# TJUMMG/OCPG

Hardware: AMD Instinct MI355X
Metric: clips/sec fwd+bwd (5x384x640, R101) (higher is better)
Workload: dtype bf16

## Files before the change

include/ocpg_hip.h:

```cpp
#ifndef OCPG_HIP_H
#define OCPG_HIP_H
#include <stdint.h>

#ifdef __cplusplus
extern "C" {
#endif

int ocpg_msda_fwd_f32(const float* value, const int64_t* shapes, const int64_t* level_start,
                      const float* loc, const float* attn,
                      int N, int S, int M, int D, int L, int Lq, int P,
                      float* out, const int64_t* shapes_host, void* stream);
int ocpg_msda_fwd_f64(const double* value, const int64_t* shapes, const int64_t* level_start,
                      const double* loc, const double* attn,
                      int N, int S, int M, int D, int L, int Lq, int P,
                      double* out, void* stream);

int ocpg_msda_bwd_f32(const float* value, const int64_t* shapes, const int64_t* level_start,
                      const float* loc, const float* attn, const float* grad_out,
                      int N, int S, int M, int D, int L, int Lq, int P,
                      float* grad_value, float* grad_loc, float* grad_attn,
                      const int64_t* shapes_host, void* stream);
int ocpg_msda_bwd_value_f32(const float* loc, const float* attn, const float* grad_out,
                            int N, int S, int M, int D, int L, int Lq, int P,
                            float* grad_value, const int64_t* shapes_host, void* stream);
int ocpg_msda_bwd_locattn_f32(const float* value, const int64_t* shapes, const int64_t* level_start,
                              const float* loc, const float* attn, const float* grad_out,
                              int N, int S, int M, int D, int L, int Lq, int P,
                              float* grad_loc, float* grad_attn, void* stream);
int ocpg_msda_fused_fwd_f32(const float* value, const int64_t* shapes, const int64_t* level_start,
                            const float* qproj, const float* ref,
                            int N, int S, int M, int D, int L, int Lq, int P,
                            float* out, float* loc_out, float* attn_out, void* stream);
int ocpg_msda_fused_bwd_qproj_f32(const float* value, const int64_t* shapes, const int64_t* level_start,
                                  const float* loc, const float* attn, const float* grad_out,
                                  int N, int S, int M, int D, int L, int Lq, int P,
                                  float* grad_qproj, void* stream);
int ocpg_msda_bwd_value_sel_f32(const float* loc, const float* attn, const float* grad_out,
                                int N, int S, int M, int D, int L, int Lq, int P,
                                float* grad_value, const int64_t* shapes_host, int* sel_state, void* stream);
int ocpg_msda_bwd_f64(const double* value, const int64_t* shapes, const int64_t* level_start,
                      const double* loc, const double* attn, const double* grad_out,
                      int N, int S, int M, int D, int L, int Lq, int P,
                      double* grad_value, double* grad_loc, double* grad_attn, void* stream);

int ocpg_msda_fwd_h16(const void* value, const int64_t* shapes, const int64_t* level_start,
                      const float* loc, const float* attn,
                      int N, int S, int M, int D, int L, int Lq, int P,
                      void* out, const int64_t* shapes_host, int dtype, void* stream);
int ocpg_msda_bwd_h16(const void* value, const int64_t* shapes, const int64_t* level_start,
                      const float* loc, const float* attn, const void* grad_out,
                      int N, int S, int M, int D, int L, int Lq, int P,
                      float* grad_value, float* grad_loc, float* grad_attn,
                      const int64_t* shapes_host, int* sel_state, int dtype, void* stream);
int ocpg_msda_bwd_value_h16(const float* loc, const float* attn, const void* grad_out,
                            int N, int S, int M, int D, int L, int Lq, int P,
                            float* grad_value, const int64_t* shapes_host, int* sel_state, int dtype, void* stream);
int ocpg_msda_bwd_locattn_h16(const void* value, const int64_t* shapes, const int64_t* level_start,
                              const float* loc, const float* attn, const void* grad_out,
                              int N, int S, int M, int D, int L, int Lq, int P,
                              float* grad_loc, float* grad_attn, int dtype, void* stream);
int ocpg_msda_fused_fwd_h16(const void* value, const int64_t* shapes, const int64_t* level_start,
                            const float* qproj, const float* ref,
                            int N, int S, int M, int D, int L, int Lq, int P,
                            void* out, float* loc_out, float* attn_out, int dtype, void* stream);
int ocpg_msda_fused_bwd_qproj_h16(const void* value, const int64_t* shapes, const int64_t* level_start,
                                  const float* loc, const float* attn, const void* grad_out,
                                  int N, int S, int M, int D, int L, int Lq, int P,
                                  float* grad_qproj, int dtype, void* stream);

int ocpg_bn_act_fwd(const void* x, const float* scale, const float* shift, const void* skip, void* y,
                    long long n_outer, int C, long long inner, int relu, int dtype, void* stream);
int ocpg_bn_act_bwd(const void* gy, const void* y, const float* scale, void* gx, void* gskip,
                    long long n_outer, int C, long long inner, int relu, int dtype, void* stream);

int ocpg_gemm_dgrad_bn_tile(long long M, int N, int K);
int ocpg_gemm_dgrad_bn(const void* a, const void* w, const void* c, const void* mask, const float* scale, void* out, void* out_skip,
                       long long M, int N, int K, int dtype, int tile, void* stream);

int ocpg_win_attn_fwd(const void* qkv, const float* biasT, const int* region, float scale, int BW, int NW, int N, int H,
                      int head_dim, void* out, float* lse, int dtype, void* stream);
int ocpg_win_attn_bwd(const void* qkv, const float* bias, const float* biasT, const int* region, float scale, int BW, int NW,
                      int N, int H, int head_dim, const void* out, const void* dout, const float* lse, void* dqkv, float* Dbuf,
                      float* dbiasT, int dtype, void* stream);

int ocpg_win_attn_bwd_mfma(const void* qkv, const float* bias, const float* biasT, const int* region, float scale, int BW, int NW, int N,
                           int H, int head_dim, const void* out, const void* dout, const float* lse, void* dqkv, float* Dbuf, void* dS,
                           int dtype, void* stream);

int ocpg_win_attn_dtable_supported(int N, int head_dim, int dtype, int T);
int ocpg_win_attn_bwd_mfma_dtable(const void* qkv, const float* bias, const float* biasT, const int* region, float scale, int BW, int NW,
                                  int N, int H, int head_dim, const void* out, const void* dout, const float* lse, void* dqkv, float* Dbuf,
                                  const int* tok_code, int code_off, int T, float* partials, float* dtable, int dtype, void* stream);

int ocpg_dynmask_fwd_f32(const float* feats, const float* params, const float* refpix, int BT, int Q, int C, int H, int W,
                         int stride, float* out, float* pre1, void* stream);

int ocpg_dynmask_bwd_pre_f32(const float* dout, const float* pre1, const float* params, int BT, int Q, int C, int H, int W,
                             int stride, float* dpre, float* part, float* w0d, void* stream);
int ocpg_dynmask_bwd_fin_f32(const float* part, const float* params, const float* refpix, const float* dw0, int BT, int Q, int C,
                             int H, int W, float* dparams, float* dref, void* stream);

int ocpg_im2col3x3_nhwc(const void* x, int N, int H, int W, int C, int stride, int dil, void* cols, int dtype, void* stream);
int ocpg_col2im3x3_nhwc(const void* dcols, int N, int H, int W, int C, int stride, int dil, void* dx, int dtype, void* stream);

int ocpg_conv3x3_mfma_fwd(const void* x, const void* w, const float* scale, const float* bias, int relu, int N, int H, int W,
                          int Cin, int Cout, int stride, void* y, void* stream);
int ocpg_conv3x3_mfma_fwd_cols(const void* x, const void* w, const float* scale, const float* bias, int relu, int N, int H, int W, int Cin,
                               int Cout, int stride, void* y, void* cols, void* stream);
int ocpg_conv3x3_mfma_dgrad(const void* dy, const void* wT, int N, int H, int W, int Cin, int Cout, int stride, void* dx,
                            void* stream);
int ocpg_conv3x3_mfma_dgrad_masked(const void* dy, const void* wT, const void* mask_y, const float* scale, int N, int H, int W, int Cin,
                                   int Cout, int stride, void* dx, void* stream);
int ocpg_conv3x3_mfma_dgrad_w(const void* dy, const void* w, const void* mask_y, const float* scale, int N, int H, int W, int Cin, int Cout,
                              int stride, void* dx, void* stream);
int ocpg_conv3x3_mfma_body_splits(long long M, int ncols, int kchannels);
int ocpg_conv3x3_mfma_fwd_bn_splitk(const void* x, const void* w, const float* scale, const float* shift, int relu, int N, int H, int W, int Cin,
                                    int Cout, int stride, int splits, float* part, void* y, void* stream);
int ocpg_conv3x3_mfma_dgrad_w_splitk(const void* dy, const void* w, const void* mask_y, const float* scale, int N, int H, int W, int Cin,
                                     int Cout, int stride, int splits, float* part, void* dx, void* stream);
int ocpg_conv3x3_mfma_wgrad_splits(int N, int H, int W, int Cin, int Cout, int stride);
int ocpg_conv3x3_mfma_wgrad(const void* gz, const void* x, int N, int H, int W, int Cin, int Cout, int stride, void* part, void* stream);
int ocpg_conv3x3_mfma_fwd_cols_h16(const void* x, const void* w, const float* scale, const float* bias, int relu, int N, int H, int W, int Cin,
                                   int Cout, int stride, void* y, void* cols, int dtype, void* stream);
int ocpg_conv3x3_mfma_dgrad_w_h16(const void* dy, const void* w, const void* mask_y, const float* scale, int N, int H, int W, int Cin, int Cout,
                                  int stride, void* dx, int dtype, void* stream);
int ocpg_conv3x3_mfma_wgrad_h16(const void* gz, const void* x, int N, int H, int W, int Cin, int Cout, int stride, void* part, int dtype,
                                void* stream);

int ocpg_conv3x3_mfma_splits(int N, int H, int W, int Cin, int Cout, int stride);
int ocpg_conv3x3_mfma_fwd_splitk(const void* x, const void* w, const float* bias, int N, int H, int W, int Cin, int Cout, int stride,
                                 int splits, float* part, void* y, int out_dt, void* cols, void* stream);
int ocpg_conv3x3_mfma_fwd_splitk_h16(const void* x, const void* w, const float* bias, int N, int H, int W, int Cin, int Cout, int stride,
                                     int splits, float* part, void* y, int out_dt, void* cols, int dtype, void* stream);

int ocpg_gemm(const void* A, const void* B, void* C, const void* bias, int dtype, int out_dtype, int transA, int transB,
              long long M, long long N, long long K, long long lda, long long ldb, long long ldc, long long batch,
              long long strideA, long long strideB, long long strideC, float alpha, float beta, void* stream);
long long ocpg_gemm_plans(void);
long long ocpg_gemm_tuned(long long* changed);
long long ocpg_gemm_tune_rejected(void);
void ocpg_gemm_set_tuning(int on);
long long ocpg_gemm_export_picks(long long* buf, long long cap_pairs);
int ocpg_gemm_import_picks(const long long* buf, long long n_pairs);
int ocpg_gemm_bn_act(const void* A, const void* W, void* D, const float* scale, const float* shift, const void* skip, int relu, int dtype,
                     long long M, long long N, long long K, void* stream);

int ocpg_levelset_fwd_f32(const float* x, const float* feats, const float* box, int Lr, int N, int C, int CF, int h, int w, float* sums,
                          float* coef, float* loss, void* stream);
int ocpg_levelset_bwd_f32(const float* x, const float* feats, const float* box, const float* coef, const float* gloss, int Lr, int N,
                          int C, int CF, int h, int w, float* gx, float* gfeat, void* stream);
int ocpg_proj_fwd_f32(const float* x, const float* tcmax, const float* trmax, const float* tcmean, const float* trmean, int Lr, int B,
                      int T, int H, int W, float* colstat, float* rowstat, float* IU, float* loss, void* stream);
int ocpg_proj_bwd_f32(const float* x, const float* tcmax, const float* trmax, const float* tcmean, const float* trmean,
                      const float* colstat, const float* rowstat, const float* IU, const float* gloss, int Lr, int B, int T, int H, int W,
                      float* Gc, float* Gr, float* gx, void* stream);

int ocpg_matcher_cost_f32(const float* logits, const float* boxes, const float* masks, long long sl, long long sb, long long st,
                          long long sq, const float* gt, const float* tboxes, const float* valid, const long long* labels, int Lr,
                          int B, int T, int Q, int K, int h, int w, float wc, float wb, float wg, float wm, float wd, float* sums,
                          float* cost, int* bad, void* stream);

int ocpg_dropout_add_ln_fwd(const void* x, const float* res, const float* gamma, const float* beta, long long R, int C, float eps, float p,
                            unsigned long long seed, unsigned long long offset, const unsigned long long* rng_base, int x_dtype, float* y,
                            float* mean, float* rstd, void* stream);
int ocpg_dropout_add_ln_bwd(const float* gy, const void* x, const float* res, const float* gamma, const float* mean, const float* rstd,
                            long long R, int C, float p, unsigned long long seed, unsigned long long offset, const unsigned long long* rng_base,
                            int x_dtype, void* gx, float* gres, float* dgb_part, void* stream);
long long ocpg_dropout_add_ln_bwd_slots(long long R);
int ocpg_bias_relu_dropout_fwd(const void* a, const void* bias, long long R, int C, float p, unsigned long long seed,
                               unsigned long long offset, const unsigned long long* rng_base, int dtype, void* h, void* stream);
int ocpg_bias_relu_dropout_bwd(const void* gh, const void* h, long long R, int C, float p, int dtype, void* ga, float* dbias_part,
                               void* stream);
long long ocpg_bias_relu_dropout_bwd_slots(long long R, int C, int dtype);

int ocpg_multi_cast(const long long* srcs, const long long* dsts, const long long* numels, const long long* chunk_prefix, int n,
                    long long total_chunks, int src_dtype, int dst_dtype, void* stream);
int ocpg_multi_cast_sum(const long long* srcs, const long long* dsts, const long long* numels, const long long* chunk_prefix,
                        const long long* splits, const long long* strides, int n, long long total_chunks, int src_dtype, int dst_dtype,
                        void* stream);
long long ocpg_colsum_blocks(long long R);
int ocpg_colsum_partials(const void* x, long long R, int C, int dtype, float* part, void* stream);

int ocpg_grad_norm_clip(const long long* grads, const long long* numels, const long long* chunk_prefix, int n, long long total_chunks,
                        float max_norm, float* partials, float* norm_and_coef, void* stream);
int ocpg_adamw_step(const long long* params, const long long* grads, const long long* exp_avg, const long long* exp_avg_sq,
                    const long long* numels, const long long* chunk_prefix, const float* lr, const float* weight_decay, int n,
                    long long total_chunks, const float* norm_and_coef, double beta1, double beta2, double eps, long long step, void* stream);
int ocpg_grad_norm_clip_amp(const long long* grads, const long long* numels, const long long* chunk_prefix, int n, long long total_chunks,
                            float max_norm, float* partials, const float* grad_scale, const float* found_inf, double beta1, double beta2,
                            float* amp_state, void* stream);
int ocpg_adamw_step_amp(const long long* params, const long long* grads, const long long* exp_avg, const long long* exp_avg_sq,
                        const long long* numels, const long long* chunk_prefix, const float* lr, const float* weight_decay, int n,
                        long long total_chunks, const float* amp_state, double beta1, double beta2, double eps, void* stream);

int ocpg_det_loss_fwd_f32(const float* logits, const float* boxes, const long long* src, const float* valid, const long long* labels,
                          const float* tboxes, const float* num_boxes, float alpha, int Lr, int B, int T, int Q, int K, float* loss, int* bad,
                          void* stream);
int ocpg_det_loss_bwd_f32(const float* logits, const float* boxes, const long long* src, const float* valid, const long long* labels,
                          const float* tboxes, const float* num_boxes, const float* gloss, float alpha, int Lr, int B, int T, int Q, int K,
                          float* glogits, float* gboxes, void* stream);

int ocpg_spectral_gate_fwd(const void* X, const float* coef, const float* high, int N, int C, int hw, float* out, void* stream);
int ocpg_spectral_c2p(const void* X, const float* coef, const float* high, int N, int C, int hw, void* pair, int dtype, void* stream);
int ocpg_spectral_p2c(const void* pair, const void* Xs, const float* coef, const float* high, int N, int C, int hw, void* out, float* part,
                      int dtype, void* stream);
int ocpg_spectral_gate_bwd(const float* gout, const void* X, const float* coef, const float* high, int N, int C, int hw, void* dX, float* part,
                           void* stream);

int ocpg_masked_ce_fwd_f32(const float* x, const float* w, const float* t, int Lr, long long per_layer, float* part, void* stream);
int ocpg_masked_ce_bwd_f32(const float* x, const float* w, const float* t, const float* gloss, int Lr, long long per_layer, float* gx,
                           void* stream);

int ocpg_attn_smallk_fwd(const void* q, long long ldq, const void* k, long long ldk, const void* v, long long ldv,
                         const unsigned char* key_pad, float scale, int Lq, int B, int H, int hd, int Lk, float pdrop,
                         unsigned long long seed, unsigned long long offset, const unsigned long long* rng_base, void* out,
                         long long ldo, float* lse, int dtype, void* stream);
int ocpg_attn_smallk_bwd(const void* q, long long ldq, const void* k, long long ldk, const void* v, long long ldv,
                         const unsigned char* key_pad, const void* dout, long long ldo, const float* lse, float scale, int Lq,
                         int B, int H, int hd, int Lk, float pdrop, unsigned long long seed, unsigned long long offset,
                         const unsigned long long* rng_base, void* dq, long long lddq, float* dk, float* dv, int dtype, void* stream);

int ocpg_lfm_dft_supported(int H, int W);
int ocpg_lfm_dft_split(int L);
int ocpg_lfm_spectrum_fwd(const float* x, const float* coef, const float* high, int N, int H, int W, int C, const void* tw_h, const void* tw_w,
                          float norm, void* tmp, void* pair, int pair_dt, void* stream);
int ocpg_lfm_spectrum_inv(const void* pair, int pair_dt, const float* coef, const float* high, const void* z_saved, float* coef_part, int N, int H,
                          int W, int C, const void* tw_h, const void* tw_w, float norm, void* tmp, const float* residual, float* out, void* stream);
int ocpg_window_means3x3_fwd(const float* x, long long planes, int h, int w, int as_bf16, float* out, void* stream);
int ocpg_window_means3x3_bwd(const float* gm, long long planes, int h, int w, float* dx, void* stream);
int ocpg_window_sums3x3_cl_bands(int h);
int ocpg_window_sums3x3_cl(const float* x, int N, int h, int w, int C, int as_bf16, float* part, void* stream);
int ocpg_window_means3x3_bwd_cl(const float* gm, int N, int h, int w, int C, const float* addend, float* dx, void* stream);

int ocpg_mso_conv3x3(const void* in, int in_dt, int relu_in, const void* w, int w_dt, const float* bias, const float* addend, int NA,
                     const void* mask, int mask_dt, const float* residual, void* out, int out_dt, int NB, int H, int W, int C,
                     int co_total, int compute_dt, void* stream);
int ocpg_mso_wgrad_rows(int NB, int H, int C, int compute_dt);
int ocpg_mso_wgrad(const void* x, int x_dt, int relu_in, const float* g, float* part, float* part_bias, int accumulate, int NB, int H, int W,
                   int C, int co, int rows_per_band, int compute_dt, void* stream);
int ocpg_bilinear_nhwc_fwd(const float* in, int NB, int H, int W, int C, int HO, int WO, float* out, void* stream);
int ocpg_bilinear_nhwc_bwd(const float* gout, int NB, int H, int W, int C, int HO, int WO, float* gin, void* stream);

int ocpg_small_linear_fwd(const void* x, int x_f32, const void* w, const void* b, int R, int Cin, int Cout, int relu, void* y, void* stream);
int ocpg_small_linear_bwd(const void* gy, int gy_f32, const void* x, int x_f32, const void* w, const void* y_relu, int R, int Cin, int Cout,
                          void* gx, void* gw, void* gb, void* stream);
int ocpg_small_linear_fwd_h16(const void* x, int x_f32, const void* w, const void* b, int R, int Cin, int Cout, int relu, void* y, int dtype,
                              void* stream);
int ocpg_small_linear_bwd_h16(const void* gy, int gy_f32, const void* x, int x_f32, const void* w, const void* y_relu, int R, int Cin, int Cout,
                              void* gx, void* gw, void* gb, int dtype, void* stream);
int ocpg_small_linear_f32_fwd(const float* x, const float* w, const float* b, int R, int Cin, int Cout, float* y, void* stream);
int ocpg_small_linear_f32_bwd(const float* gy, const float* x, const float* w, int R, int Cin, int Cout, float* gx, float* gw, float* gb, void* stream);

int ocpg_layernorm_blocks(long long rows);
int ocpg_layernorm_fwd(const void* x, int x_f32, const float* gamma, const float* beta, long long rows, int C, float eps, void* y, int y_f32,
                       float* mean, float* rstd, void* stream);
int ocpg_layernorm_bwd(const void* gy, int gy_f32, const void* x, int x_f32, const float* gamma, const float* mean, const float* rstd,
                       long long rows, int C, void* dx, int dx_f32, float* part_g, float* part_b, void* stream);

long long ocpg_groupnorm_cl_work(long long N, int HW, int C, int G);
int ocpg_groupnorm_cl_fwd(const void* x, int x_dtype, const float* gamma, const float* beta, long long N, int HW, int C, int G, float eps,
                          float* y, float* mean, float* rstd, float* work, void* stream);
int ocpg_groupnorm_cl_bwd(const float* gy, const void* x, int x_dtype, const float* gamma, const float* mean, const float* rstd, long long N,
                          int HW, int C, int G, void* dx, float* part, float* work, void* stream);
int ocpg_groupnorm_cl2cl_fwd(const void* x, int x_dtype, const float* gamma, const float* beta, long long N, int HW, int C, int G, float eps,
                             float* y, float* mean, float* rstd, float* work, void* stream);
int ocpg_groupnorm_cl2cl_bwd(const float* gy, const void* x, int x_dtype, const float* gamma, const float* mean, const float* rstd, long long N,
                             int HW, int C, int G, void* dx, float* part, float* work, void* stream);

int ocpg_gather_rows_bwd(const float* g, const long long* order, const long long* seg, int T, int H, float* out, void* stream);
int ocpg_relpos_bias_fwd(const float* table, const long long* idx, int N, long long ldi, int H, float* bias, float* bias_t, void* stream);
int ocpg_relpos_bias_bwd(const float* g, const long long* order, const long long* seg, int T, int H, int N, int transposed, float* out,
                         void* stream);

int ocpg_gather_rows_pad(const void* x, const long long* idx, long long B, long long S, long long M, long long row_bytes, void* out,
                         void* stream);

int ocpg_graph_replace_memsets(void* hip_graph, int* n_replaced);
int ocpg_graph_stats(void* hip_graph, long long* out9);
int ocpg_graph_memcpy_nodes(void* hip_graph, long long* out, int cap);

const char* ocpg_hip_version(void);

#ifdef __cplusplus
}
#endif
#endif
```

ocpg_amd/_lib.py:

```python
import ctypes
import os

import torch

_HERE = os.path.dirname(os.path.abspath(__file__))
LIB_PATH = os.environ.get("OCPG_HIP_LIB") or os.path.join(_HERE, "lib", "libocpg_hip.so")
_lib = None

_i64p = ctypes.c_void_p
_vp = ctypes.c_void_p
_int = ctypes.c_int

SIGNATURES = {
    "ocpg_msda_fwd_f32": [_vp, _i64p, _i64p, _vp, _vp] + [_int] * 7 + [_vp, _vp, _vp],
    "ocpg_msda_fwd_f64": [_vp, _i64p, _i64p, _vp, _vp] + [_int] * 7 + [_vp, _vp],
    "ocpg_msda_bwd_f32": [_vp, _i64p, _i64p, _vp, _vp, _vp] + [_int] * 7 + [_vp, _vp, _vp, _vp, _vp],
    "ocpg_msda_bwd_value_f32": [_vp, _vp, _vp] + [_int] * 7 + [_vp, _vp, _vp],
    "ocpg_msda_fused_fwd_f32": [_vp, _i64p, _i64p, _vp, _vp] + [_int] * 7 + [_vp, _vp, _vp, _vp],
    "ocpg_msda_fused_bwd_qproj_f32": [_vp, _i64p, _i64p, _vp, _vp, _vp] + [_int] * 7 + [_vp, _vp],
    "ocpg_msda_bwd_value_sel_f32": [_vp, _vp, _vp] + [_int] * 7 + [_vp, _vp, _vp, _vp],
    "ocpg_msda_bwd_locattn_f32": [_vp, _i64p, _i64p, _vp, _vp, _vp] + [_int] * 7 + [_vp, _vp, _vp],
    "ocpg_msda_bwd_f64": [_vp, _i64p, _i64p, _vp, _vp, _vp] + [_int] * 7 + [_vp, _vp, _vp, _vp],
    "ocpg_msda_fwd_h16": [_vp, _i64p, _i64p, _vp, _vp] + [_int] * 7 + [_vp, _vp, _int, _vp],
    "ocpg_msda_bwd_h16": [_vp, _i64p, _i64p, _vp, _vp, _vp] + [_int] * 7 + [_vp, _vp, _vp, _vp, _vp, _int, _vp],
    "ocpg_msda_bwd_value_h16": [_vp, _vp, _vp] + [_int] * 7 + [_vp, _vp, _vp, _int, _vp],
    "ocpg_msda_bwd_locattn_h16": [_vp, _i64p, _i64p, _vp, _vp, _vp] + [_int] * 7 + [_vp, _vp, _int, _vp],
    "ocpg_msda_fused_fwd_h16": [_vp, _i64p, _i64p, _vp, _vp] + [_int] * 7 + [_vp, _vp, _vp, _int, _vp],
    "ocpg_msda_fused_bwd_qproj_h16": [_vp, _i64p, _i64p, _vp, _vp, _vp] + [_int] * 7 + [_vp, _int, _vp],
    "ocpg_bn_act_fwd": [_vp, _vp, _vp, _vp, _vp, ctypes.c_longlong, _int, ctypes.c_longlong, _int, _int, _vp],
    "ocpg_bn_act_bwd": [_vp, _vp, _vp, _vp, _vp, ctypes.c_longlong, _int, ctypes.c_longlong, _int, _int, _vp],
    "ocpg_gemm_dgrad_bn_tile": [ctypes.c_longlong, _int, _int],
    "ocpg_gemm_dgrad_bn": [_vp] * 7 + [ctypes.c_longlong, _int, _int, _int, _int, _vp],
    "ocpg_dynmask_fwd_f32": [_vp, _vp, _vp] + [_int] * 6 + [_vp, _vp, _vp],
    "ocpg_dynmask_bwd_pre_f32": [_vp, _vp, _vp] + [_int] * 6 + [_vp, _vp, _vp, _vp],
    "ocpg_dynmask_bwd_fin_f32": [_vp, _vp, _vp, _vp] + [_int] * 5 + [_vp, _vp, _vp],
    "ocpg_conv3x3_mfma_fwd": [_vp, _vp, _vp, _vp] + [_int] * 7 + [_vp, _vp],
    "ocpg_conv3x3_mfma_fwd_cols": [_vp, _vp, _vp, _vp] + [_int] * 7 + [_vp, _vp, _vp],
    "ocpg_conv3x3_mfma_dgrad": [_vp, _vp] + [_int] * 6 + [_vp, _vp],
    "ocpg_conv3x3_mfma_dgrad_masked": [_vp, _vp, _vp, _vp] + [_int] * 6 + [_vp, _vp],
    "ocpg_conv3x3_mfma_dgrad_w": [_vp, _vp, _vp, _vp] + [_int] * 6 + [_vp, _vp],
    "ocpg_conv3x3_mfma_splits": [_int] * 6,
    "ocpg_conv3x3_mfma_wgrad_splits": [_int] * 6,
    "ocpg_conv3x3_mfma_body_splits": [ctypes.c_longlong, _int, _int],
    "ocpg_conv3x3_mfma_fwd_bn_splitk": [_vp, _vp, _vp, _vp] + [_int] * 8 + [_vp, _vp, _vp],
    "ocpg_conv3x3_mfma_dgrad_w_splitk": [_vp, _vp, _vp, _vp] + [_int] * 7 + [_vp, _vp, _vp],
    "ocpg_conv3x3_mfma_wgrad": [_vp, _vp] + [_int] * 6 + [_vp, _vp],
    "ocpg_conv3x3_mfma_fwd_cols_h16": [_vp, _vp, _vp, _vp] + [_int] * 7 + [_vp, _vp, _int, _vp],
    "ocpg_conv3x3_mfma_dgrad_w_h16": [_vp, _vp, _vp, _vp] + [_int] * 6 + [_vp, _int, _vp],
    "ocpg_conv3x3_mfma_wgrad_h16": [_vp, _vp] + [_int] * 6 + [_vp, _int, _vp],
    "ocpg_conv3x3_mfma_fwd_splitk": [_vp, _vp, _vp] + [_int] * 7 + [_vp, _vp, _int, _vp, _vp],
    "ocpg_conv3x3_mfma_fwd_splitk_h16": [_vp, _vp, _vp] + [_int] * 7 + [_vp, _vp, _int, _vp, _int, _vp],
    "ocpg_gemm": [_vp, _vp, _vp, _vp] + [_int] * 4 + [ctypes.c_longlong] * 10 + [ctypes.c_float, ctypes.c_float, _vp],
    "ocpg_gemm_plans": [],
    "ocpg_gemm_tuned": [_vp],
    "ocpg_gemm_tune_rejected": [],
    "ocpg_gemm_set_tuning": [_int],
    "ocpg_gemm_export_picks": [_vp, ctypes.c_longlong],
    "ocpg_gemm_import_picks": [_vp, ctypes.c_longlong],
    "ocpg_window_means3x3_fwd": [_vp, ctypes.c_longlong, _int, _int, _int, _vp, _vp],
    "ocpg_window_means3x3_bwd": [_vp, ctypes.c_longlong, _int, _int, _vp, _vp],
    "ocpg_window_sums3x3_cl_bands": [_int],
    "ocpg_window_sums3x3_cl": [_vp, _int, _int, _int, _int, _int, _vp, _vp],
    "ocpg_window_means3x3_bwd_cl": [_vp, _int, _int, _int, _int, _vp, _vp, _vp],
    "ocpg_mso_conv3x3": [_vp, _int, _int, _vp, _int, _vp, _vp, _int, _vp, _int, _vp, _vp, _int] + [_int] * 6 + [_vp],
    "ocpg_mso_wgrad_rows": [_int] * 4,
    "ocpg_mso_wgrad": [_vp, _int, _int, _vp, _vp, _vp] + [_int] * 8 + [_vp],
    "ocpg_bilinear_nhwc_fwd": [_vp] + [_int] * 6 + [_vp, _vp],
    "ocpg_bilinear_nhwc_bwd": [_vp] + [_int] * 6 + [_vp, _vp],
    "ocpg_small_linear_fwd": [_vp, _int, _vp, _vp, _int, _int, _int, _int, _vp, _vp],
    "ocpg_small_linear_bwd": [_vp, _int, _vp, _int, _vp, _vp, _int, _int, _int, _vp, _vp, _vp, _vp],
    "ocpg_small_linear_fwd_h16": [_vp, _int, _vp, _vp, _int, _int, _int, _int, _vp, _int, _vp],
    "ocpg_small_linear_bwd_h16": [_vp, _int, _vp, _int, _vp, _vp, _int, _int, _int, _vp, _vp, _vp, _int, _vp],
    "ocpg_small_linear_f32_fwd": [_vp, _vp, _vp, _int, _int, _int, _vp, _vp],
    "ocpg_small_linear_f32_bwd": [_vp, _vp, _vp, _int, _int, _int, _vp, _vp, _vp, _vp],
    "ocpg_layernorm_blocks": [ctypes.c_longlong],
    "ocpg_groupnorm_cl_work": [ctypes.c_longlong, _int, _int, _int],
    "ocpg_groupnorm_cl_fwd": [_vp, _int, _vp, _vp, ctypes.c_longlong, _int, _int, _int, ctypes.c_float, _vp, _vp, _vp, _vp, _vp],
    "ocpg_groupnorm_cl_bwd": [_vp, _vp, _int, _vp, _vp, _vp, ctypes.c_longlong, _int, _int, _int, _vp, _vp, _vp, _vp],
    "ocpg_groupnorm_cl2cl_fwd": [_vp, _int, _vp, _vp, ctypes.c_longlong, _int, _int, _int, ctypes.c_float, _vp, _vp, _vp, _vp, _vp],
    "ocpg_groupnorm_cl2cl_bwd": [_vp, _vp, _int, _vp, _vp, _vp, ctypes.c_longlong, _int, _int, _int, _vp, _vp, _vp, _vp],
    "ocpg_layernorm_fwd": [_vp, _int, _vp, _vp, ctypes.c_longlong, _int, ctypes.c_float, _vp, _int, _vp, _vp, _vp],
    "ocpg_layernorm_bwd": [_vp, _int, _vp, _int, _vp, _vp, _vp, ctypes.c_longlong, _int, _vp, _int, _vp, _vp, _vp],
    "ocpg_gather_rows_bwd": [_vp, _vp, _vp, _int, _int, _vp, _vp],
    "ocpg_relpos_bias_fwd": [_vp, _vp, _int, ctypes.c_longlong, _int, _vp, _vp, _vp],
    "ocpg_relpos_bias_bwd": [_vp, _vp, _vp, _int, _int, _int, _int, _vp, _vp],
    "ocpg_gather_rows_pad": [_vp, _vp] + [ctypes.c_longlong] * 4 + [_vp, _vp],
    "ocpg_graph_replace_memsets": [_vp, _vp],
    "ocpg_graph_stats": [_vp, _vp],
    "ocpg_graph_memcpy_nodes": [_vp, _vp, _int],
    "ocpg_gemm_bn_act": [_vp] * 6 + [_int, _int] + [ctypes.c_longlong] * 3 + [_vp],
    "ocpg_levelset_fwd_f32": [_vp] * 3 + [_int] * 6 + [_vp] * 4,
    "ocpg_levelset_bwd_f32": [_vp] * 5 + [_int] * 6 + [_vp] * 3,
    "ocpg_proj_fwd_f32": [_vp] * 5 + [_int] * 5 + [_vp] * 5,
    "ocpg_proj_bwd_f32": [_vp] * 9 + [_int] * 5 + [_vp] * 4,
    "ocpg_matcher_cost_f32": [_vp] * 3 + [ctypes.c_longlong] * 4 + [_vp] * 4 + [_int] * 7 + [ctypes.c_float] * 5 + [_vp] * 4,
    "ocpg_dropout_add_ln_fwd": [_vp] * 4 + [ctypes.c_longlong, _int, ctypes.c_float, ctypes.c_float, ctypes.c_ulonglong, ctypes.c_ulonglong, _vp, _int]
                               + [_vp] * 4,
    "ocpg_dropout_add_ln_bwd": [_vp] * 6 + [ctypes.c_longlong, _int, ctypes.c_float, ctypes.c_ulonglong, ctypes.c_ulonglong, _vp, _int] + [_vp] * 4,
    "ocpg_dropout_add_ln_bwd_slots": [ctypes.c_longlong],
    "ocpg_bias_relu_dropout_fwd": [_vp, _vp, ctypes.c_longlong, _int, ctypes.c_float, ctypes.c_ulonglong, ctypes.c_ulonglong, _vp, _int, _vp, _vp],
    "ocpg_bias_relu_dropout_bwd": [_vp, _vp, ctypes.c_longlong, _int, ctypes.c_float, _int, _vp, _vp, _vp],
    "ocpg_bias_relu_dropout_bwd_slots": [ctypes.c_longlong, _int, _int],
    "ocpg_multi_cast": [_vp] * 4 + [_int, ctypes.c_longlong, _int, _int, _vp],
    "ocpg_multi_cast_sum": [_vp] * 6 + [_int, ctypes.c_longlong, _int, _int, _vp],
    "ocpg_colsum_blocks": [ctypes.c_longlong],
    "ocpg_grad_norm_clip": [_vp] * 3 + [_int, ctypes.c_longlong, ctypes.c_float, _vp, _vp, _vp],
    "ocpg_adamw_step": [_vp] * 8 + [_int, ctypes.c_longlong, _vp, ctypes.c_double, ctypes.c_double, ctypes.c_double, ctypes.c_longlong, _vp],
    "ocpg_grad_norm_clip_amp": [_vp] * 3 + [_int, ctypes.c_longlong, ctypes.c_float, _vp, _vp, _vp, ctypes.c_double, ctypes.c_double, _vp, _vp],
    "ocpg_adamw_step_amp": [_vp] * 8 + [_int, ctypes.c_longlong, _vp, ctypes.c_double, ctypes.c_double, ctypes.c_double, _vp],
    "ocpg_lfm_dft_supported": [_int, _int],
    "ocpg_lfm_dft_split": [_int],
    "ocpg_lfm_spectrum_fwd": [_vp, _vp, _vp] + [_int] * 4 + [_vp, _vp, ctypes.c_float, _vp, _vp, _int, _vp],
    "ocpg_lfm_spectrum_inv": [_vp, _int, _vp, _vp, _vp, _vp] + [_int] * 4 + [_vp, _vp, ctypes.c_float, _vp, _vp, _vp, _vp],
    "ocpg_colsum_partials": [_vp, ctypes.c_longlong, _int, _int, _vp, _vp],
    "ocpg_det_loss_fwd_f32": [_vp] * 7 + [ctypes.c_float] + [_int] * 5 + [_vp] * 3,
    "ocpg_det_loss_bwd_f32": [_vp] * 8 + [ctypes.c_float] + [_int] * 5 + [_vp] * 3,
    "ocpg_spectral_gate_fwd": [_vp] * 3 + [_int] * 3 + [_vp, _vp],
    "ocpg_spectral_gate_bwd": [_vp] * 4 + [_int] * 3 + [_vp, _vp, _vp],
    "ocpg_spectral_c2p": [_vp] * 3 + [_int] * 3 + [_vp, _int, _vp],
    "ocpg_spectral_p2c": [_vp] * 4 + [_int] * 3 + [_vp, _vp, _int, _vp],
    "ocpg_masked_ce_fwd_f32": [_vp] * 3 + [_int, ctypes.c_longlong, _vp, _vp],
    "ocpg_masked_ce_bwd_f32": [_vp] * 4 + [_int, ctypes.c_longlong, _vp, _vp],
    "ocpg_im2col3x3_nhwc": [_vp] + [_int] * 6 + [_vp, _int, _vp],
    "ocpg_col2im3x3_nhwc": [_vp] + [_int] * 6 + [_vp, _int, _vp],
    "ocpg_attn_smallk_fwd": [_vp, ctypes.c_longlong, _vp, ctypes.c_longlong, _vp, ctypes.c_longlong, _vp, ctypes.c_float] + [_int] * 5
                            + [ctypes.c_float, ctypes.c_ulonglong, ctypes.c_ulonglong, _vp, _vp, ctypes.c_longlong, _vp, _int, _vp],
    "ocpg_attn_smallk_bwd": [_vp, ctypes.c_longlong, _vp, ctypes.c_longlong, _vp, ctypes.c_longlong, _vp, _vp, ctypes.c_longlong, _vp,
                             ctypes.c_float] + [_int] * 5 + [ctypes.c_float, ctypes.c_ulonglong, ctypes.c_ulonglong, _vp, _vp, ctypes.c_longlong,
                                                             _vp, _vp, _int, _vp],
    "ocpg_win_attn_fwd": [_vp, _vp, _vp, ctypes.c_float] + [_int] * 5 + [_vp, _vp, _int, _vp],
    "ocpg_win_attn_bwd": [_vp, _vp, _vp, _vp, ctypes.c_float] + [_int] * 5 + [_vp] * 6 + [_int, _vp],
    "ocpg_win_attn_bwd_mfma": [_vp, _vp, _vp, _vp, ctypes.c_float] + [_int] * 5 + [_vp] * 6 + [_int, _vp],
    "ocpg_win_attn_dtable_supported": [_int] * 4,
    "ocpg_win_attn_bwd_mfma_dtable": [_vp, _vp, _vp, _vp, ctypes.c_float] + [_int] * 5 + [_vp] * 6 + [_int, _int, _vp, _vp, _int, _vp],
}


_TIMING = {"on": False, "events": []}
_UNTIMED = ("ocpg_win_attn_dtable_supported", "ocpg_conv3x3_mfma_body_splits", "ocpg_gemm_dgrad_bn_tile", "ocpg_conv3x3_mfma_wgrad_splits", "ocpg_window_sums3x3_cl_bands", "ocpg_lfm_dft_supported", "ocpg_lfm_dft_split", "ocpg_conv3x3_mfma_splits", "ocpg_gemm_set_tuning", "ocpg_gemm_export_picks", "ocpg_gemm_import_picks", "ocpg_colsum_blocks", "ocpg_mso_wgrad_rows", "ocpg_gemm_plans", "ocpg_gemm_tuned", "ocpg_gemm_tune_rejected", "ocpg_bias_relu_dropout_bwd_slots", "ocpg_dropout_add_ln_bwd_slots", "ocpg_groupnorm_cl_work")


def enable_kernel_timing(on=True):
    _TIMING["on"] = on
    _TIMING["events"] = []


def collect_kernel_timing(work=None):
    torch.cuda.synchronize()
    out = {}
    for name, args, e0, e1 in _TIMING["events"]:
        d = out.setdefault(name, {"ms": 0.0, "n": 0, "work": 0.0, "modelled": 0})
        d["ms"] += e0.elapsed_time(e1)
        d["n"] += 1
        w = work(name, args) if work is not None else None
        if isinstance(w, tuple):
            d["work_lowp"] = d.get("work_lowp", 0.0) + (w[0] if w[1] else 0.0)
            w = w[0]
        if w is not None:
            d["work"] += w
            d["modelled"] += 1
    _TIMING["events"] = []
    _TIMING["on"] = False
    return out


CENSUS = {"on": False, "calls": {}}


def census(on=True):
    CENSUS["on"] = on
    if on:
        CENSUS["calls"] = {}
    return CENSUS["calls"]


class _Lib:

    def __init__(self, cdll):
        self._cdll = cdll

    def __getattr__(self, name):
        fn = getattr(self._cdll, name)
        if name not in SIGNATURES or name in _UNTIMED:
            setattr(self, name, fn)
            return fn
        timed = not name.startswith("ocpg_msda_")

        def call(*a):
            if CENSUS["on"]:
                rc = fn(*a)
                if rc == 0:
                    CENSUS["calls"][name] = CENSUS["calls"].get(name, 0) + 1
                return rc
            if not (timed and _TIMING["on"]):
                return fn(*a)
            e0, e1 = torch.cuda.Event(enable_timing=True), torch.cuda.Event(enable_timing=True)
            e0.record()
            rc = fn(*a)
            e1.record()
            _TIMING["events"].append((name, tuple(getattr(x, "value", x) for x in a), e0, e1))
            return rc
        setattr(self, name, call)
        return call


def lib():
    global _lib
    if _lib is None:
        if not os.path.exists(LIB_PATH):
            raise RuntimeError(
                f"{LIB_PATH} not found: build it with `python -m ocpg_amd.csrc.build` "
                "(hipcc --offload-arch=gfx950). The HIP extension is mandatory; there is no CPU/PyTorch fallback.")
        L = ctypes.CDLL(LIB_PATH)
        for name, argtypes in SIGNATURES.items():
            fn = getattr(L, name)
            fn.argtypes = argtypes
            fn.restype = ctypes.c_int
        L.ocpg_hip_version.restype = ctypes.c_char_p
        L.ocpg_gemm_plans.restype = ctypes.c_longlong
        L.ocpg_gemm_tuned.restype = ctypes.c_longlong
        L.ocpg_gemm_tune_rejected.restype = ctypes.c_longlong
        L.ocpg_gemm_export_picks.restype = ctypes.c_longlong
        L.ocpg_gemm_set_tuning.restype = None
        L.ocpg_bias_relu_dropout_bwd_slots.restype = ctypes.c_longlong
        L.ocpg_dropout_add_ln_bwd_slots.restype = ctypes.c_longlong
        L.ocpg_groupnorm_cl_work.restype = ctypes.c_longlong
        L.ocpg_colsum_blocks.restype = ctypes.c_longlong
        _lib = _Lib(L)
    return _lib


def check(status, what):
    if status != 0:
        if status <= -1000:
            raise RuntimeError(f"{what}: invalid argument #{-status - 1000}")
        raise RuntimeError(f"{what}: HIP error {-status}")


def stream_ptr():
    return ctypes.c_void_p(torch.cuda.current_stream().cuda_stream)


def require_gpu(name, t):
    if not t.is_cuda:
        raise RuntimeError(f"{name} must be a GPU tensor: Not implemented on the CPU")
    if not t.is_contiguous():
        raise RuntimeError(f"{name} tensor has to be contiguous")
```

ocpg_amd/csrc/conv3x3_mfma.hip:

```cpp
#include <hip/hip_bf16.h>
#include <hip/hip_fp16.h>
#include <hip/hip_runtime.h>
#include <stdint.h>

#include <cstdlib>

#include "../../include/ocpg_hip.h"
#include "conv3x3_halo.h"
#include "h16_elem.h"

namespace {

typedef ocpg_h16::h16x8 bf16x8;
typedef ocpg_h16::f32x16 f32x16;

struct Bf16 : ocpg_h16::Bf16 { static constexpr bool STATIC_TAIL = false; };
struct Fp16 : ocpg_h16::Fp16 { static constexpr bool STATIC_TAIL = true; };

constexpr int BM = 64, BK = 64, NT = 256;
constexpr int LDS_ROW = BK + 8;
constexpr int SEGS = BK / 8;
constexpr int ROWS_PER_PASS = NT / SEGS;
constexpr int A_L = BM / ROWS_PER_PASS;
constexpr int NSETS = 3;

struct ConvGeom {
  int N, H, W, C;
  int Hs, Ws;
  int Cout;
  int stride;
  long long M;
};

template <bool DGRAD>
__device__ __forceinline__ bool tap_source(const ConvGeom& g, int y, int x, int ky, int kx, int& ys, int& xs) {
  if (!DGRAD) {
    ys = y * g.stride + ky - 1;
    xs = x * g.stride + kx - 1;
    return ys >= 0 && ys < g.Hs && xs >= 0 && xs < g.Ws;
  } else {
    const int ty = y + 1 - ky, tx = x + 1 - kx;
    if (ty < 0 || tx < 0 || (g.stride == 2 && ((ty | tx) & 1))) return false;
    ys = g.stride == 2 ? ty >> 1 : ty;
    xs = g.stride == 2 ? tx >> 1 : tx;
    return ys < g.Hs && xs < g.Ws;
  }
}

#define CONV3X3_KERNEL conv3x3_mfma
#define CONV3X3_ELEM Bf16
#include "conv3x3_mfma_kernel.h"
#undef CONV3X3_KERNEL
#undef CONV3X3_ELEM
#define CONV3X3_KERNEL conv3x3_mfma_f16
#define CONV3X3_ELEM Fp16
#include "conv3x3_mfma_kernel.h"
#undef CONV3X3_KERNEL
#undef CONV3X3_ELEM

inline bool narrow_tiles(unsigned mtiles, int ncols) {
  static const int mode = [] { const char* e = std::getenv("OCPG_CONV3X3_BN"); return e ? std::atoi(e) : 0; }();
  if (mode == 64) return true;
  if (mode == 128) return false;
  return (long long)mtiles * ((ncols + 127) / 128) < 3 * 256;
}

inline bool halo_variant() {
  static const bool on = [] { const char* e = std::getenv("OCPG_CONV3X3_HALO"); return e && e[0] == '1'; }();
  return on;
}

}

extern "C" int ocpg_conv3x3_mfma_fwd_cols_h16(const void* x, const void* w, const float* scale, const float* bias, int relu, int N, int H, int W,
                                              int Cin, int Cout, int stride, void* y, void* cols, int dtype, void* stream) {
  if (dtype != 1 && dtype != 2) return -1010;
  if (N < 0 || H <= 0 || W <= 0 || Cin <= 0 || Cout <= 0) return -1006;
  if ((stride != 1 && stride != 2) || Cin % BK != 0) return -2000;
  if (N == 0) return 0;
  if (!x) return -1001;
  if (!w) return -1002;
  if (!y) return -1010;
  if (dtype == 1 && stride == 1 && !cols && halo_variant() &&
      ocpg_halo::conv3x3_halo((const __hip_bfloat16*)x, (const __hip_bfloat16*)w, scale, bias, relu, 0, N, H, W, Cin, Cout, (__hip_bfloat16*)y,
                              (hipStream_t)stream)) {
    const hipError_t e = hipGetLastError();
    return e == hipSuccess ? 0 : -(int)e;
  }
  ConvGeom g;
  g.N = N; g.H = (H - 1) / stride + 1; g.W = (W - 1) / stride + 1; g.C = Cin; g.Hs = H; g.Ws = W; g.Cout = Cout; g.stride = stride;
  g.M = (long long)N * g.H * g.W;
  const unsigned mt = (unsigned)((g.M + BM - 1) / BM);
  const bool narrow = narrow_tiles(mt, Cout);
  const dim3 grid(mt, (unsigned)(narrow ? (Cout + 63) / 64 : (Cout + 127) / 128));
  if (dtype == 2) {
    if (narrow)
      conv3x3_mfma_f16<false, 64><<<grid, NT, 0, (hipStream_t)stream>>>((const __half*)x, (const __half*)w, scale, bias, relu, g, (__half*)y, (__half*)cols);
    else
      conv3x3_mfma_f16<false, 128><<<grid, NT, 0, (hipStream_t)stream>>>((const __half*)x, (const __half*)w, scale, bias, relu, g, (__half*)y, (__half*)cols);
  } else if (narrow) {
    conv3x3_mfma<false, 64><<<grid, NT, 0, (hipStream_t)stream>>>(
        (const __hip_bfloat16*)x, (const __hip_bfloat16*)w, scale, bias, relu, g, (__hip_bfloat16*)y, (__hip_bfloat16*)cols);
  } else {
    conv3x3_mfma<false, 128><<<grid, NT, 0, (hipStream_t)stream>>>(
        (const __hip_bfloat16*)x, (const __hip_bfloat16*)w, scale, bias, relu, g, (__hip_bfloat16*)y, (__hip_bfloat16*)cols);
  }
  const hipError_t e = hipGetLastError();
  return e == hipSuccess ? 0 : -(int)e;
}

extern "C" int ocpg_conv3x3_mfma_fwd_cols(const void* x, const void* w, const float* scale, const float* bias, int relu, int N, int H, int W,
                                          int Cin, int Cout, int stride, void* y, void* cols, void* stream) {
  return ocpg_conv3x3_mfma_fwd_cols_h16(x, w, scale, bias, relu, N, H, W, Cin, Cout, stride, y, cols, 1, stream);
}

extern "C" int ocpg_conv3x3_mfma_fwd(const void* x, const void* w, const float* scale, const float* bias, int relu, int N, int H, int W,
                                     int Cin, int Cout, int stride, void* y, void* stream) {
  return ocpg_conv3x3_mfma_fwd_cols(x, w, scale, bias, relu, N, H, W, Cin, Cout, stride, y, nullptr, stream);
}

extern "C" int ocpg_conv3x3_mfma_dgrad_masked(const void* dy, const void* wT, const void* mask_y, const float* scale, int N, int H, int W, int Cin,
                                              int Cout, int stride, void* dx, void* stream);
extern "C" int ocpg_conv3x3_mfma_dgrad(const void* dy, const void* wT, int N, int H, int W, int Cin, int Cout, int stride, void* dx,
                                       void* stream) {
  return ocpg_conv3x3_mfma_dgrad_masked(dy, wT, nullptr, nullptr, N, H, W, Cin, Cout, stride, dx, stream);
}

extern "C" int ocpg_conv3x3_mfma_dgrad_masked(const void* dy, const void* wT, const void* mask_y, const float* scale, int N, int H, int W, int Cin,
                                              int Cout, int stride, void* dx, void* stream) {
  if (N < 0 || H <= 0 || W <= 0 || Cin <= 0 || Cout <= 0) return -1006;
  if ((stride != 1 && stride != 2) || Cout % BK != 0) return -2000;
  if (N == 0) return 0;
  if (!dy) return -1001;
  if (!wT) return -1002;
  if (!dx) return -1009;
  if (stride == 1 && !mask_y && !scale && halo_variant() &&
      ocpg_halo::conv3x3_halo((const __hip_bfloat16*)dy, (const __hip_bfloat16*)wT, nullptr, nullptr, 0, 1, N, H, W, Cout, Cin, (__hip_bfloat16*)dx,
                              (hipStream_t)stream)) {
    const hipError_t e = hipGetLastError();
    return e == hipSuccess ? 0 : -(int)e;
  }
  ConvGeom g;
  g.N = N; g.H = H; g.W = W; g.C = Cout; g.Hs = (H - 1) / stride + 1; g.Ws = (W - 1) / stride + 1; g.Cout = Cin; g.stride = stride;
  g.M = (long long)N * H * W;
  const unsigned mt = (unsigned)((g.M + BM - 1) / BM);
  if (narrow_tiles(mt, Cin))
    conv3x3_mfma<true, 64><<<dim3(mt, (unsigned)((Cin + 63) / 64)), NT, 0, (hipStream_t)stream>>>(
        (const __hip_bfloat16*)dy, (const __hip_bfloat16*)wT, scale, nullptr, 0, g, (__hip_bfloat16*)dx, nullptr, (const __hip_bfloat16*)mask_y);
  else
    conv3x3_mfma<true, 128><<<dim3(mt, (unsigned)((Cin + 127) / 128)), NT, 0, (hipStream_t)stream>>>(
        (const __hip_bfloat16*)dy, (const __hip_bfloat16*)wT, scale, nullptr, 0, g, (__hip_bfloat16*)dx, nullptr, (const __hip_bfloat16*)mask_y);
  const hipError_t e = hipGetLastError();
  return e == hipSuccess ? 0 : -(int)e;
}

extern "C" int ocpg_conv3x3_mfma_dgrad_w_h16(const void* dy, const void* w, const void* mask_y, const float* scale, int N, int H, int W, int Cin,
                                             int Cout, int stride, void* dx, int dtype, void* stream) {
  if (dtype != 1 && dtype != 2) return -1010;
  if (N < 0 || H <= 0 || W <= 0 || Cin <= 0 || Cout <= 0) return -1006;
  if ((stride != 1 && stride != 2) || Cout % BK != 0 || Cin % 8 != 0) return -2000;
  if (N == 0) return 0;
  if (!dy) return -1001;
  if (!w) return -1002;
  if (!dx) return -1011;
  ConvGeom g;
  g.N = N; g.H = H; g.W = W; g.C = Cout; g.Hs = (H - 1) / stride + 1; g.Ws = (W - 1) / stride + 1; g.Cout = Cin; g.stride = stride;
  g.M = (long long)N * H * W;
  const unsigned mt = (unsigned)((g.M + BM - 1) / BM);
  const bool narrow = narrow_tiles(mt, Cin);
  const dim3 grid(mt, (unsigned)(narrow ? (Cin + 63) / 64 : (Cin + 127) / 128));
  if (dtype == 2) {
    if (narrow)
      conv3x3_mfma_f16<true, 64, false, true><<<grid, NT, 0, (hipStream_t)stream>>>((const __half*)dy, (const __half*)w, scale, nullptr, 0, g, (__half*)dx, nullptr,
                                                                             (const __half*)mask_y);
    else
      conv3x3_mfma_f16<true, 128, false, true><<<grid, NT, 0, (hipStream_t)stream>>>((const __half*)dy, (const __half*)w, scale, nullptr, 0, g, (__half*)dx, nullptr,
                                                                              (const __half*)mask_y);
  } else if (narrow) {
    conv3x3_mfma<true, 64, false, true><<<grid, NT, 0, (hipStream_t)stream>>>(
        (const __hip_bfloat16*)dy, (const __hip_bfloat16*)w, scale, nullptr, 0, g, (__hip_bfloat16*)dx, nullptr, (const __hip_bfloat16*)mask_y);
  } else {
    conv3x3_mfma<true, 128, false, true><<<grid, NT, 0, (hipStream_t)stream>>>(
        (const __hip_bfloat16*)dy, (const __hip_bfloat16*)w, scale, nullptr, 0, g, (__hip_bfloat16*)dx, nullptr, (const __hip_bfloat16*)mask_y);
  }
  const hipError_t e = hipGetLastError();
  return e == hipSuccess ? 0 : -(int)e;
}

extern "C" int ocpg_conv3x3_mfma_dgrad_w(const void* dy, const void* w, const void* mask_y, const float* scale, int N, int H, int W, int Cin, int Cout,
                                         int stride, void* dx, void* stream) {
  return ocpg_conv3x3_mfma_dgrad_w_h16(dy, w, mask_y, scale, N, H, W, Cin, Cout, stride, dx, 1, stream);
}

namespace {

__global__ __launch_bounds__(256) void k_splitk_reduce(const float* __restrict__ part, const float* __restrict__ bias, int splits, long long MC, int Cout,
                                                       void* __restrict__ out, int out_dt, const float* __restrict__ scale = nullptr, int relu = 0,
                                                       const __hip_bfloat16* __restrict__ mask = nullptr) {
  const long long i = ((long long)blockIdx.x * 256 + threadIdx.x) * 4;
  if (i >= MC) return;
  float4 a = make_float4(0.f, 0.f, 0.f, 0.f);
  for (int z = 0; z < splits; ++z) {
    const float4 v = *reinterpret_cast<const float4*>(part + (long long)z * MC + i);
    a.x += v.x; a.y += v.y; a.z += v.z; a.w += v.w;
  }
  const int c = (int)(i % Cout);
  if (scale) {
    const float4 sv = *reinterpret_cast<const float4*>(scale + c);
    a.x *= sv.x; a.y *= sv.y; a.z *= sv.z; a.w *= sv.w;
  }
  if (bias) {
    const float4 bv = *reinterpret_cast<const float4*>(bias + c);
    a.x += bv.x; a.y += bv.y; a.z += bv.z; a.w += bv.w;
  }
  if (relu) { a.x = fmaxf(a.x, 0.f); a.y = fmaxf(a.y, 0.f); a.z = fmaxf(a.z, 0.f); a.w = fmaxf(a.w, 0.f); }
  if (mask) {
    const ushort4 mk = *reinterpret_cast<const ushort4*>(reinterpret_cast<const unsigned short*>(mask) + i);
    if (!((short)mk.x > 0)) a.x = 0.f;
    if (!((short)mk.y > 0)) a.y = 0.f;
    if (!((short)mk.z > 0)) a.z = 0.f;
    if (!((short)mk.w > 0)) a.w = 0.f;
  }
  if (out_dt == 0) {
    *reinterpret_cast<float4*>(reinterpret_cast<float*>(out) + i) = a;
  } else if (out_dt == 2) {
    ushort4 o;
    o.x = ocpg_h16::Fp16::bits(a.x); o.y = ocpg_h16::Fp16::bits(a.y); o.z = ocpg_h16::Fp16::bits(a.z); o.w = ocpg_h16::Fp16::bits(a.w);
    *reinterpret_cast<ushort4*>(reinterpret_cast<unsigned short*>(out) + i) = o;
  } else {
    ushort4 o;
    o.x = __bfloat16_as_ushort(__float2bfloat16(a.x)); o.y = __bfloat16_as_ushort(__float2bfloat16(a.y));
    o.z = __bfloat16_as_ushort(__float2bfloat16(a.z)); o.w = __bfloat16_as_ushort(__float2bfloat16(a.w));
    *reinterpret_cast<ushort4*>(reinterpret_cast<unsigned short*>(out) + i) = o;
  }
}

}

extern "C" int ocpg_conv3x3_mfma_splits(int N, int H, int W, int Cin, int Cout, int stride) {
  if (N <= 0 || H <= 0 || W <= 0 || Cin <= 0 || Cout <= 0 || (stride != 1 && stride != 2) || Cin % BK != 0 || Cout % 4 != 0) return 1;
  const long long M = (long long)N * ((H - 1) / stride + 1) * ((W - 1) / stride + 1);
  const long long tiles = ((M + BM - 1) / BM) * ((Cout + 63) / 64);
  const int chunks = Cin / BK;
  int best = 1;
  for (int sgl = 1; sgl <= chunks; ++sgl)
    if (chunks % sgl == 0 && chunks / sgl >= 2 && tiles * sgl <= 1024) best = sgl;
  return tiles < 256 ? best : 1;
}

extern "C" int ocpg_conv3x3_mfma_fwd_splitk_h16(const void* x, const void* w, const float* bias, int N, int H, int W, int Cin, int Cout, int stride,
                                                int splits, float* part, void* y, int out_dt, void* cols, int dtype, void* stream) {
  if (dtype != 1 && dtype != 2) return -1010;
  if (N < 0 || H <= 0 || W <= 0 || Cin <= 0 || Cout <= 0) return -1006;
  if ((stride != 1 && stride != 2) || Cin % BK != 0 || Cout % 4 != 0 || splits < 1 || (Cin / BK) % splits != 0 || (out_dt != 0 && out_dt != dtype)) return -2000;
  if (N == 0) return 0;
  if (!x) return -1001;
  if (!w) return -1002;
  if (!part) return -1011;
  if (!y) return -1012;
  ConvGeom g;
  g.N = N; g.H = (H - 1) / stride + 1; g.W = (W - 1) / stride + 1; g.C = Cin; g.Hs = H; g.Ws = W; g.Cout = Cout; g.stride = stride;
  g.M = (long long)N * g.H * g.W;
  const unsigned mt = (unsigned)((g.M + BM - 1) / BM);
  const dim3 grid(mt, (unsigned)((Cout + 63) / 64), (unsigned)splits);
  if (dtype == 2)
    conv3x3_mfma_f16<false, 64, true><<<grid, NT, 0, (hipStream_t)stream>>>((const __half*)x, (const __half*)w, nullptr, nullptr, 0, g,
                                                                          reinterpret_cast<__half*>(part), (__half*)cols);
  else
    conv3x3_mfma<false, 64, true><<<grid, NT, 0, (hipStream_t)stream>>>(
        (const __hip_bfloat16*)x, (const __hip_bfloat16*)w, nullptr, nullptr, 0, g, reinterpret_cast<__hip_bfloat16*>(part), (__hip_bfloat16*)cols);
  const long long MC = g.M * Cout;
  k_splitk_reduce<<<(unsigned)((MC / 4 + 255) / 256), 256, 0, (hipStream_t)stream>>>(part, bias, splits, MC, Cout, y, out_dt);
  const hipError_t e = hipGetLastError();
  return e == hipSuccess ? 0 : -(int)e;
}

extern "C" int ocpg_conv3x3_mfma_fwd_splitk(const void* x, const void* w, const float* bias, int N, int H, int W, int Cin, int Cout, int stride,
                                            int splits, float* part, void* y, int out_dt, void* cols, void* stream) {
  return ocpg_conv3x3_mfma_fwd_splitk_h16(x, w, bias, N, H, W, Cin, Cout, stride, splits, part, y, out_dt, cols, 1, stream);
}

extern "C" int ocpg_conv3x3_mfma_body_splits(long long M, int ncols, int kchannels) {
  if (M <= 0 || ncols <= 0 || kchannels <= 0 || kchannels % BK != 0 || ncols % 4 != 0) return 1;
  static const int mode = [] { const char* e = std::getenv("OCPG_CONV3X3_SPLITK"); return e ? std::atoi(e) : -1; }();
  const long long tiles = ((M + BM - 1) / BM) * ((ncols + 63) / 64);
  const int chunks = kchannels / BK;
  if (mode == 0) return 1;
  if (mode > 1) return chunks % mode == 0 ? mode : 1;
  if (tiles > 640) return 1;
  int best = 1;
  for (int sgl = 2; sgl <= chunks; ++sgl)
    if (chunks % sgl == 0 && chunks / sgl >= 2 && tiles * sgl <= 1280) best = sgl;
  return best;
}

extern "C" int ocpg_conv3x3_mfma_fwd_bn_splitk(const void* x, const void* w, const float* scale, const float* shift, int relu, int N, int H, int W, int Cin,
                                               int Cout, int stride, int splits, float* part, void* y, void* stream) {
  if (N < 0 || H <= 0 || W <= 0 || Cin <= 0 || Cout <= 0) return -1006;
  if ((stride != 1 && stride != 2) || Cin % BK != 0 || Cout % 4 != 0 || splits < 2 || (Cin / BK) % splits != 0) return -2000;
  if (N == 0) return 0;
  if (!x) return -1001;
  if (!w) return -1002;
  if (!part) return -1013;
  if (!y) return -1014;
  ConvGeom g;
  g.N = N; g.H = (H - 1) / stride + 1; g.W = (W - 1) / stride + 1; g.C = Cin; g.Hs = H; g.Ws = W; g.Cout = Cout; g.stride = stride;
  g.M = (long long)N * g.H * g.W;
  const unsigned mt = (unsigned)((g.M + BM - 1) / BM);
  conv3x3_mfma<false, 64, true><<<dim3(mt, (unsigned)((Cout + 63) / 64), (unsigned)splits), NT, 0, (hipStream_t)stream>>>(
      (const __hip_bfloat16*)x, (const __hip_bfloat16*)w, nullptr, nullptr, 0, g, reinterpret_cast<__hip_bfloat16*>(part), nullptr);
  const long long MC = g.M * Cout;
  k_splitk_reduce<<<(unsigned)((MC / 4 + 255) / 256), 256, 0, (hipStream_t)stream>>>(part, shift, splits, MC, Cout, y, 1, scale, relu);
  const hipError_t e = hipGetLastError();
  return e == hipSuccess ? 0 : -(int)e;
}

extern "C" int ocpg_conv3x3_mfma_dgrad_w_splitk(const void* dy, const void* w, const void* mask_y, const float* scale, int N, int H, int W, int Cin,
                                                int Cout, int stride, int splits, float* part, void* dx, void* stream) {
  if (N < 0 || H <= 0 || W <= 0 || Cin <= 0 || Cout <= 0) return -1006;
  if ((stride != 1 && stride != 2) || Cout % BK != 0 || Cin % 8 != 0 || splits < 2 || (Cout / BK) % splits != 0) return -2000;
  if (N == 0) return 0;
  if (!dy) return -1001;
  if (!w) return -1002;
  if (!part) return -1012;
  if (!dx) return -1013;
  ConvGeom g;
  g.N = N; g.H = H; g.W = W; g.C = Cout; g.Hs = (H - 1) / stride + 1; g.Ws = (W - 1) / stride + 1; g.Cout = Cin; g.stride = stride;
  g.M = (long long)N * H * W;
  const unsigned mt = (unsigned)((g.M + BM - 1) / BM);
  conv3x3_mfma<true, 64, true, true><<<dim3(mt, (unsigned)((Cin + 63) / 64), (unsigned)splits), NT, 0, (hipStream_t)stream>>>(
      (const __hip_bfloat16*)dy, (const __hip_bfloat16*)w, nullptr, nullptr, 0, g, reinterpret_cast<__hip_bfloat16*>(part), nullptr);
  const long long MC = g.M * Cin;
  k_splitk_reduce<<<(unsigned)((MC / 4 + 255) / 256), 256, 0, (hipStream_t)stream>>>(part, nullptr, splits, MC, Cin, dx, 1, scale, 0, (const __hip_bfloat16*)mask_y);
  const hipError_t e = hipGetLastError();
  return e == hipSuccess ? 0 : -(int)e;
}
```

ocpg_amd/csrc/conv3x3_mfma_kernel.h:

```cpp
template <bool DGRAD, int BN, bool SPLITK = false, bool BTR = false>
__global__ __launch_bounds__(NT) void CONV3X3_KERNEL(const CONV3X3_ELEM::T* __restrict__ x, const CONV3X3_ELEM::T* __restrict__ w,
                                                     const float* __restrict__ scale, const float* __restrict__ bias, int relu, ConvGeom g,
                                                     CONV3X3_ELEM::T* __restrict__ y, CONV3X3_ELEM::T* __restrict__ cols,
                                                     const CONV3X3_ELEM::T* __restrict__ mask = nullptr) {
  using E = CONV3X3_ELEM;
  using T = E::T;
  static_assert(!SPLITK || BN == 64, "the split-K epilogue is the 64-column one");
  static_assert(!BTR || DGRAD, "the untransposed weight operand is the input gradient's");
  constexpr int BROW = BN + 8;
  constexpr int BSEG = BN / 8;
  static_assert(BK * BROW <= BN * LDS_ROW, "the [k][n] image fits the [n][k] one's buffer");
  constexpr int B_L = BN / ROWS_PER_PASS, NJ = BN / 64, WN = BN / 2;
  constexpr bool KSPLIT = BN == 64;
  constexpr int NACC = KSPLIT ? 4 : NJ;
  __shared__ __attribute__((aligned(16))) short smem[2 * BM * LDS_ROW + 2 * BN * LDS_ROW];
  short (*As)[BM * LDS_ROW] = reinterpret_cast<short (*)[BM * LDS_ROW]>(smem);
  short (*Bs)[BN * LDS_ROW] = reinterpret_cast<short (*)[BN * LDS_ROW]>(smem + 2 * BM * LDS_ROW);
  const int tid = threadIdx.x, lane = tid & 63, wave = tid >> 6;
  const int wm = wave & 1, wn = wave >> 1;
  const long long m0 = (long long)blockIdx.x * BM;
  const int n0 = blockIdx.y * BN;
  const int srow = tid / SEGS, sseg = tid % SEGS;
  int pn[A_L], py[A_L], px[A_L];
  bool row_ok[A_L];
  {
    const int hw = g.H * g.W;
#pragma unroll
    for (int i = 0; i < A_L; ++i) {
      const long long mrow = m0 + srow + i * ROWS_PER_PASS;
      row_ok[i] = mrow < g.M;
      const long long mr = row_ok[i] ? mrow : 0;
      pn[i] = (int)(mr / hw);
      const int r = (int)(mr - (long long)pn[i] * hw);
      py[i] = r / g.W;
      px[i] = r - py[i] * g.W;
    }
  }
  const int C = g.C, ksteps_per_tap = C / BK;
  const int cps = SPLITK ? ksteps_per_tap / (int)gridDim.z : ksteps_per_tap;
  const int c_lo = SPLITK ? (int)blockIdx.z * cps : 0, c_hi = c_lo + cps;
  const int ksteps = 9 * cps;
  const long long wrow_stride = 9LL * C;
  const T* wp[B_L];
#pragma unroll
  for (int i = 0; i < B_L; ++i) {
    if constexpr (BTR) {
      const int e = tid + i * NT, kr = e / BSEG, ns = e % BSEG;
      wp[i] = w + (long long)kr * (9LL * g.Cout) + min(n0 + ns * 8, g.Cout - 8);
    } else {
      wp[i] = w + (long long)min(n0 + srow + i * ROWS_PER_PASS, g.Cout - 1) * wrow_stride + sseg * 8;
    }
  }

  struct Regs { uint4 a[A_L], b[B_L]; unsigned z; int coff; };
  Regs S0, S1;
  int f_tap = 0, f_c = c_lo;
  auto fetch = [&](Regs& R) {
    uint4 (&a)[A_L] = R.a; uint4 (&bq)[B_L] = R.b; unsigned& z = R.z;
    const int tap = f_tap, fc = min(f_c, c_hi - 1);
    const int ky = (tap * 11) >> 5, kx = tap - ky * 3;
    const int c0 = fc * BK + sseg * 8;
    R.coff = f_c < c_hi ? tap * C + c0 : -1;
    z = 0;
#pragma unroll
    for (int i = 0; i < A_L; ++i) {
      int ys = 0, xs = 0;
      const bool ok = row_ok[i] && tap_source<DGRAD>(g, py[i], px[i], ky, kx, ys, xs);
      if (!ok) { ys = 0; xs = 0; z |= 1u << i; }
      a[i] = *reinterpret_cast<const uint4*>(x + (((long long)pn[i] * g.Hs + ys) * g.Ws + xs) * C + c0);
    }
    const long long woff = BTR ? (long long)fc * BK * (9LL * g.Cout) + (long long)tap * g.Cout : (long long)tap * C + fc * BK;
#pragma unroll
    for (int i = 0; i < B_L; ++i) bq[i] = *reinterpret_cast<const uint4*>(wp[i] + woff);
    if (++f_tap == 9) { f_tap = 0; ++f_c; }
  };
  auto park = [&](int buf, const Regs& R) {
    const uint4 (&a)[A_L] = R.a; const uint4 (&bq)[B_L] = R.b; const unsigned z = R.z;
#pragma unroll
    for (int i = 0; i < A_L; ++i)
      *reinterpret_cast<uint4*>(&As[buf][(srow + i * ROWS_PER_PASS) * LDS_ROW + sseg * 8]) = ((z >> i) & 1u) ? make_uint4(0u, 0u, 0u, 0u) : a[i];
#pragma unroll
    for (int i = 0; i < B_L; ++i) {
      if constexpr (BTR) {
        const int e = tid + i * NT;
        *reinterpret_cast<uint4*>(&Bs[buf][(e / BSEG) * BROW + (e % BSEG) * 8]) = bq[i];
      } else {
        *reinterpret_cast<uint4*>(&Bs[buf][(srow + i * ROWS_PER_PASS) * LDS_ROW + sseg * 8]) = bq[i];
      }
    }
    if constexpr (!DGRAD) {
      if (cols && blockIdx.y == 0 && R.coff >= 0) {
#pragma unroll
        for (int i = 0; i < A_L; ++i)
          if (row_ok[i])
            *reinterpret_cast<uint4*>(cols + (m0 + srow + i * ROWS_PER_PASS) * (9LL * C) + R.coff) = ((z >> i) & 1u) ? make_uint4(0u, 0u, 0u, 0u) : a[i];
      }
    }
  };

  f32x16 acc[NACC];
#pragma unroll
  for (int i = 0; i < NACC; ++i)
#pragma unroll
    for (int r = 0; r < 16; ++r) acc[i][r] = 0.f;

  const int fr = lane & 31, fh = lane >> 5;
  auto btr = [&](int buf, int k0, int ncol0) -> bf16x8 {
    typedef short s4 __attribute__((ext_vector_type(4)));
    const int li = lane & 15, grp = lane >> 4;
    const short* p = &Bs[buf][(k0 + 8 * fh + (li >> 2)) * BROW + ncol0 + 16 * (grp & 1) + 4 * (li & 3)];
    const s4 lo = __builtin_amdgcn_ds_read_tr16_b64_v4i16((__attribute__((address_space(3))) s4*)p);
    const s4 hi = __builtin_amdgcn_ds_read_tr16_b64_v4i16((__attribute__((address_space(3))) s4*)(p + 4 * BROW));
    bf16x8 r;
    r[0] = lo[0]; r[1] = lo[1]; r[2] = lo[2]; r[3] = lo[3]; r[4] = hi[0]; r[5] = hi[1]; r[6] = hi[2]; r[7] = hi[3];
    return r;
  };
  auto compute = [&](int buf) {
    if constexpr (KSPLIT) {
      static_assert(BK / 16 == NT / 64, "one 16-wide K slice per wave");
      const int ko = wave * 16 + fh * 8;
      const bf16x8 a0 = *reinterpret_cast<const bf16x8*>(&As[buf][fr * LDS_ROW + ko]);
      const bf16x8 a1 = *reinterpret_cast<const bf16x8*>(&As[buf][(32 + fr) * LDS_ROW + ko]);
      bf16x8 b0, b1;
      if constexpr (BTR) {
        b0 = btr(buf, wave * 16, 0);
        b1 = btr(buf, wave * 16, 32);
      } else {
        b0 = *reinterpret_cast<const bf16x8*>(&Bs[buf][fr * LDS_ROW + ko]);
        b1 = *reinterpret_cast<const bf16x8*>(&Bs[buf][(32 + fr) * LDS_ROW + ko]);
      }
      acc[0] = E::mfma(a0, b0, acc[0]);
      acc[1] = E::mfma(a0, b1, acc[1]);
      acc[2] = E::mfma(a1, b0, acc[2]);
      acc[3] = E::mfma(a1, b1, acc[3]);
      return;
    }
#pragma unroll
    for (int kk = 0; kk < BK / 16; ++kk) {
      const bf16x8 a = *reinterpret_cast<const bf16x8*>(&As[buf][(wm * 32 + fr) * LDS_ROW + kk * 16 + fh * 8]);
#pragma unroll
      for (int j = 0; j < NJ; ++j) {
        bf16x8 b;
        if constexpr (BTR) b = btr(buf, kk * 16, wn * WN + j * 32);
        else b = *reinterpret_cast<const bf16x8*>(&Bs[buf][(wn * WN + j * 32 + fr) * LDS_ROW + kk * 16 + fh * 8]);
        acc[j] = E::mfma(a, b, acc[j]);
      }
    }
  };
  static_assert(NSETS == 3, "the k loop below is written for three register sets");
  Regs S2;
  fetch(S0);
  fetch(S1);
  fetch(S2);
  park(0, S0);
  fetch(S0);
  __syncthreads();
  auto step = [&](int s_, Regs& nxt) {
    park((s_ & 1) ^ 1, nxt);
    fetch(nxt);
    if (s_ < ksteps) compute(s_ & 1);
    __syncthreads();
  };
  for (int ks = 0; ks < ksteps; ks += 3) {
    step(ks, S1);
    step(ks + 1, S2);
    step(ks + 2, S0);
  }
  if constexpr (KSPLIT) {
    float* red = reinterpret_cast<float*>(smem);
    static_assert(sizeof(smem) >= 2 * 4096 * sizeof(float), "two tile images");
    auto put = [&](float* d) {
#pragma unroll
      for (int t = 0; t < 4; ++t)
#pragma unroll
        for (int r = 0; r < 16; ++r) d[(t * 16 + r) * 64 + lane] = acc[t][r];
    };
    auto add = [&](const float* d) {
#pragma unroll
      for (int t = 0; t < 4; ++t)
#pragma unroll
        for (int r = 0; r < 16; ++r) acc[t][r] += d[(t * 16 + r) * 64 + lane];
    };
    if (wave >= 2) put(red + (wave - 2) * 4096);
    __syncthreads();
    if (wave < 2) add(red + wave * 4096);
    __syncthreads();
    if (wave == 1) put(red + 4096);
    __syncthreads();
    if (wave == 0) { add(red + 4096); put(red); }
    __syncthreads();
    const int m = tid >> 2, nq = (tid & 3) * 16;
    const long long row = m0 + m;
    if (row < g.M) {
      const int r = (m & 3) + 4 * ((m & 31) >> 3), h = ((m & 31) >> 2) & 1, t0 = (m >> 5) * 2 + (nq >> 5);
      const float* src = red + (t0 * 16 + r) * 64 + (nq & 31) + 32 * h;
      const int col0 = n0 + nq;
      if constexpr (SPLITK) {
        float* dst = reinterpret_cast<float*>(y) + ((long long)blockIdx.z * g.M + row) * g.Cout + col0;
        if (col0 + 16 <= g.Cout && (g.Cout & 3) == 0) {
#pragma unroll
          for (int q = 0; q < 4; ++q) reinterpret_cast<float4*>(dst)[q] = make_float4(src[4 * q], src[4 * q + 1], src[4 * q + 2], src[4 * q + 3]);
        } else {
          for (int j = 0; j < 16 && col0 + j < g.Cout; ++j) dst[j] = src[j];
        }
        return;
      }
      short o[16];
      float sc[16], bi[16];
      const bool full = col0 + 16 <= g.Cout;
      if (full) {
#pragma unroll
        for (int q = 0; q < 4; ++q) {
          const float4 a = scale ? reinterpret_cast<const float4*>(scale + col0)[q] : make_float4(1.f, 1.f, 1.f, 1.f);
          const float4 b = bias ? reinterpret_cast<const float4*>(bias + col0)[q] : make_float4(0.f, 0.f, 0.f, 0.f);
          sc[4 * q] = a.x, sc[4 * q + 1] = a.y, sc[4 * q + 2] = a.z, sc[4 * q + 3] = a.w;
          bi[4 * q] = b.x, bi[4 * q + 1] = b.y, bi[4 * q + 2] = b.z, bi[4 * q + 3] = b.w;
        }
      } else {
#pragma unroll
        for (int j = 0; j < 16; ++j) {
          const int col = min(col0 + j, g.Cout - 1);
          sc[j] = scale ? scale[col] : 1.f;
          bi[j] = bias ? bias[col] : 0.f;
        }
      }
      bool keep[16];
#pragma unroll
      for (int j = 0; j < 16; ++j) keep[j] = true;
      if (mask) {
        const T* mk = mask + row * g.Cout + col0;
        if (full && (g.Cout & 7) == 0) {
          const bf16x8 lo = *reinterpret_cast<const bf16x8*>(mk), hi = *reinterpret_cast<const bf16x8*>(mk + 8);
#pragma unroll
          for (int j = 0; j < 8; ++j) { keep[j] = lo[j] > 0; keep[8 + j] = hi[j] > 0; }
        } else if constexpr (E::STATIC_TAIL) {
#pragma unroll
          for (int j = 0; j < 16; ++j)
            if (col0 + j < g.Cout) keep[j] = reinterpret_cast<const short*>(mk)[j] > 0;
        } else {
          for (int j = 0; j < 16 && col0 + j < g.Cout; ++j) keep[j] = reinterpret_cast<const short*>(mk)[j] > 0;
        }
      }
#pragma unroll
      for (int j = 0; j < 16; ++j) {
        float v = src[j] * sc[j] + bi[j];
        if (relu) v = fmaxf(v, 0.f);
        if (!keep[j]) v = 0.f;
        o[j] = (short)E::bits(v);
      }
      T* dst = y + row * g.Cout + col0;
      if (col0 + 16 <= g.Cout && (g.Cout & 7) == 0) {
        bf16x8 lo, hi;
#pragma unroll
        for (int j = 0; j < 8; ++j) { lo[j] = o[j]; hi[j] = o[8 + j]; }
        *reinterpret_cast<bf16x8*>(dst) = lo;
        *reinterpret_cast<bf16x8*>(dst + 8) = hi;
      } else if constexpr (E::STATIC_TAIL) {
#pragma unroll
        for (int j = 0; j < 16; ++j)
          if (col0 + j < g.Cout) reinterpret_cast<short*>(dst)[j] = o[j];
      } else {
        for (int j = 0; j < 16 && col0 + j < g.Cout; ++j) reinterpret_cast<short*>(dst)[j] = o[j];
      }
    }
    return;
  }
#pragma unroll
  for (int j = 0; j < NJ; ++j) {
    const int col = n0 + wn * WN + j * 32 + (lane & 31);
    if (col >= g.Cout) continue;
    const float sv = scale ? scale[col] : 1.f, bv = bias ? bias[col] : 0.f;
#pragma unroll
    for (int r = 0; r < 16; ++r) {
      const long long row = m0 + wm * 32 + (r & 3) + 8 * (r >> 2) + 4 * (lane >> 5);
      float v = acc[j][r] * sv + bv;
      if (relu) v = fmaxf(v, 0.f);
      if (row < g.M) {
        if (mask && !(reinterpret_cast<const short*>(mask)[row * g.Cout + col] > 0)) v = 0.f;
        y[row * g.Cout + col] = E::narrow(v);
      }
    }
  }
}
```

ocpg_amd/models/ops/functions/conv_bn_func.py:

```python
import os

import torch
from torch.autograd import Function
from torch.autograd.function import once_differentiable

from ...._lib import check, lib

_DT = {torch.float32: 0, torch.bfloat16: 1, torch.float16: 2}
_H16 = (torch.bfloat16, torch.float16)
_CL = torch.channels_last
EPILOGUE = os.environ.get("OCPG_GEMM_EPILOGUE", "1") != "0"
FWD_COLS = os.environ.get("OCPG_CONV3X3_FWD_COLS", "0") != "0"
SKIP_GRAD_IN_GEMM = os.environ.get("OCPG_SKIP_GRAD_IN_GEMM", "1") != "0"
_SKIP_TOKENS = {}
PREMASK = os.environ.get("OCPG_PREMASK_DGRAD", "1") != "0"
_PREMASK_TOKENS = {}
FUSED_DGRAD_BN = os.environ.get("OCPG_FUSED_DGRAD_BN", "1") != "0"
_DGRAD_BN_DECLINED = (-2000, -2001, -2002)


def reset_skip_tokens():
    _SKIP_TOKENS.clear()
    _PREMASK_TOKENS.clear()


def _same_tensor(a, b):
    if a is None or b is None:
        return False
    return a is b or (a.data_ptr() == b.data_ptr() and a.shape == b.shape and a.dtype == b.dtype and a.stride() == b.stride()
                      and a._version == b._version)


def _tensor_key(t):
    return (t.data_ptr(), tuple(t.shape), t.dtype, tuple(t.stride()), t._version)


def _both16(*ts):
    return ts[0].dtype in _H16 and all(t.dtype == ts[0].dtype for t in ts)


def _offer_token(y, scale, skip, switch):
    tok = {"y": _tensor_key(y), "scale": scale, "skip": skip, "switch": switch, "gz": None, "gskip": None, "ver": None}
    _PREMASK_TOKENS[y.data_ptr()] = tok
    return tok


def _claim_token(x):
    tok = _PREMASK_TOKENS.pop(x.data_ptr(), None)
    return tok if (tok is not None and tok["y"] == _tensor_key(x)) else None


def _fill_token(tok, gz, gskip=None):
    tok["gz"], tok["gskip"], tok["ver"] = gz, gskip, gz._version


def _take_token(tok, gy):
    if tok is None or tok["gz"] is None:
        return None
    gz, gskip, ver = tok["gz"], tok["gskip"], tok["ver"]
    tok["gz"] = tok["gskip"] = tok["ver"] = None
    if not (gy.data_ptr() == gz.data_ptr() and gy.shape == gz.shape and gy.stride() == gz.stride() and gy._version == ver):
        raise RuntimeError(f"{tok['switch']}=1: the gradient of this conv + BN + ReLU output was produced with the BN + ReLU backward already "
                           f"applied by its consumer's input-gradient kernel, but a different gradient arrived (a second consumer of the "
                           f"output, or a gradient hook); run with {tok['switch']}=0 for such a graph")
    return gz, gskip


def _dgrad_bn(a, w, c, mask, scale, out, out_skip, m, n, k, st):
    L = lib()
    tile = int(L.ocpg_gemm_dgrad_bn_tile(m, n, k))
    if tile < 0:
        return _DGRAD_BN_DECLINED[0]
    rc = L.ocpg_gemm_dgrad_bn(a.data_ptr(), w.data_ptr(), None if c is None else c.data_ptr(), mask.data_ptr(), scale.data_ptr(), out.data_ptr(),
                              None if out_skip is None else out_skip.data_ptr(), m, n, k, _DT.get(a.dtype, -1), tile, st)
    if rc and rc not in _DGRAD_BN_DECLINED:
        check(rc, "ocpg_gemm_dgrad_bn")
    return rc


def _reduce_partials(part, w_is_cast_copy):
    from ... import amp_cache
    if w_is_cast_copy and amp_cache.DEFER_SUM and amp_cache.MULTI_CAST and part.dtype in (torch.bfloat16, torch.float16):
        return amp_cache.defer_sum(part)
    return part.sum(0)


def eligible(x, conv):
    return (x.is_cuda and x.dim() == 4 and x.dtype in _DT and conv.kernel_size == (1, 1) and conv.stride == (1, 1) and conv.padding == (0, 0)
            and conv.groups == 1 and conv.bias is None and x.is_contiguous(memory_format=_CL))


def eligible_s2(x, conv):
    return (x.is_cuda and x.dim() == 4 and x.dtype in _DT and conv.kernel_size == (1, 1) and conv.stride == (2, 2) and conv.padding == (0, 0)
            and conv.groups == 1 and conv.bias is None and x.is_contiguous(memory_format=_CL))


class Subsample2(Function):

    @staticmethod
    def forward(ctx, x):
        ctx.shape = x.shape
        return x[:, :, ::2, ::2].contiguous(memory_format=_CL)

    @staticmethod
    @once_differentiable
    def backward(ctx, g):
        gx = torch.empty(ctx.shape, dtype=g.dtype, device=g.device, memory_format=_CL).zero_()
        gx[:, :, ::2, ::2] = g
        return gx


def subsample2(x):
    return Subsample2.apply(x)


class Conv1x1BNAct(Function):
    @staticmethod
    def forward(ctx, x, w, scale, shift, skip, relu, splits):
        n, c, h, wd = x.shape
        co = w.shape[0]
        m = n * h * wd
        dt = _DT[x.dtype]
        L = lib()
        st = torch.cuda.current_stream().cuda_stream
        y = torch.empty((n, co, h, wd), dtype=x.dtype, device=x.device, memory_format=_CL)
        if skip is not None and (skip.dtype != x.dtype or not skip.is_contiguous(memory_format=_CL)):
            skip = skip.to(x.dtype).contiguous(memory_format=_CL)
        rc = -1105
        if EPILOGUE:
            rc = L.ocpg_gemm_bn_act(x.data_ptr(), w.data_ptr(), y.data_ptr(), scale.data_ptr(), shift.data_ptr(),
                                    None if skip is None else skip.data_ptr(), int(relu), dt, m, co, c, st)
            if rc and rc != -1105:
                check(rc, "ocpg_gemm_bn_act")
        if rc:
            rc = L.ocpg_gemm(x.data_ptr(), w.data_ptr(), y.data_ptr(), None, dt, dt, 0, 1, m, co, c, c, c, co, 1, 0, 0, 0, 1.0, 0.0, st)
            if rc:
                check(rc, "ocpg_gemm")
            rc = L.ocpg_bn_act_fwd(y.data_ptr(), scale.data_ptr(), shift.data_ptr(), None if skip is None else skip.data_ptr(), y.data_ptr(),
                                   m, co, 1, int(relu), dt, st)
            if rc:
                check(rc, "ocpg_bn_act_fwd")
        ctx.save_for_backward(x, w, y, scale)
        from ...amp_cache import is_cast_copy
        ctx.meta = (bool(relu), skip is not None, splits)
        ctx.w_cast = is_cast_copy(w)
        ctx.give = ctx.take = None
        ctx.claim = _claim_token(x) if (FUSED_DGRAD_BN and _both16(x, w) and ctx.needs_input_grad[0]) else None
        ctx.premask = None
        if PREMASK and relu and skip is None and _both16(x, w) and ctx.needs_input_grad[1]:
            ctx.premask = _offer_token(y, scale, False, "OCPG_PREMASK_DGRAD")
        elif FUSED_DGRAD_BN and relu and skip is not None and _both16(x, w) and any(ctx.needs_input_grad):
            ctx.premask = _offer_token(y, scale, True, "OCPG_FUSED_DGRAD_BN")
        if SKIP_GRAD_IN_GEMM:
            if skip is not None:
                tok = _SKIP_TOKENS.pop(skip.data_ptr(), None)
                if tok is not None and _same_tensor(tok["x"], skip) and ctx.needs_input_grad[4]:
                    ctx.give = tok
            elif ctx.needs_input_grad[0]:
                ctx.take = {"x": x, "g": None}
                _SKIP_TOKENS[x.data_ptr()] = ctx.take
        return y

    @staticmethod
    @once_differentiable
    def backward(ctx, gy):
        x, w, y, scale = ctx.saved_tensors
        relu, has_skip, splits = ctx.meta
        n, c, h, wd = x.shape
        co = w.shape[0]
        m = n * h * wd
        dt = _DT[x.dtype]
        L = lib()
        st = torch.cuda.current_stream().cuda_stream
        if gy.dtype != y.dtype or not gy.is_contiguous(memory_format=_CL):
            gy = gy.to(y.dtype).contiguous(memory_format=_CL)
        need_x, need_w, need_skip = ctx.needs_input_grad[0], ctx.needs_input_grad[1], has_skip and ctx.needs_input_grad[4]
        fused = _take_token(ctx.premask, gy)
        if fused is not None:
            gz, gskip = fused
            if not need_skip:
                gskip = None
        else:
            gz = torch.empty_like(y)
            gskip = torch.empty_like(y) if need_skip else None
            rc = L.ocpg_bn_act_bwd(gy.data_ptr(), y.data_ptr(), scale.data_ptr(), gz.data_ptr(), None if gskip is None else gskip.data_ptr(),
                                   m, co, 1, int(relu), dt, st)
            if rc:
                check(rc, "ocpg_bn_act_bwd")
        gx = gw = None
        if ctx.give is not None and need_skip:
            ctx.give["g"] = gskip
            gskip = None
        parked = None
        if ctx.take is not None:
            parked, ctx.take["g"], ctx.take["x"] = ctx.take["g"], None, None
        if need_x:
            acc = parked is not None and parked.dtype == x.dtype and parked.shape == x.shape and parked.is_contiguous(memory_format=_CL)
            tok = ctx.claim
            gx = None
            if tok is not None and (parked is None or acc) and (acc or not tok["skip"]):
                gx = torch.empty((n, c, h, wd), dtype=x.dtype, device=x.device, memory_format=_CL)
                out_skip = parked if tok["skip"] else None
                if _dgrad_bn(gz, w, parked if acc else None, x, tok["scale"], gx, out_skip, m, c, co, st) == 0:
                    _fill_token(tok, gx, out_skip)
                else:
                    gx = None
            if gx is None:
                gx = parked if acc else torch.empty((n, c, h, wd), dtype=x.dtype, device=x.device, memory_format=_CL)
                rc = L.ocpg_gemm(gz.data_ptr(), w.data_ptr(), gx.data_ptr(), None, dt, dt, 0, 0, m, c, co, co, c, c, 1, 0, 0, 0, 1.0,
                                 1.0 if acc else 0.0, st)
                if rc:
                    check(rc, "ocpg_gemm")
                if parked is not None and not acc:
                    gx = gx + parked
        elif parked is not None:
            gx = parked
        if need_w:
            from ...amp_cache import side_wgrad
            with side_wgrad(ctx.w_cast, gz, x) as sw:
                st = torch.cuda.current_stream().cuda_stream
                if splits > 1 and m % splits == 0:
                    r = m // splits
                    part = torch.empty((splits, co, c), dtype=x.dtype, device=x.device)
                    rc = L.ocpg_gemm(gz.data_ptr(), x.data_ptr(), part.data_ptr(), None, dt, dt, 1, 0, co, c, r, co, c, c, splits, r * co, r * c,
                                     co * c, 1.0, 0.0, st)
                    gw = _reduce_partials(part, ctx.w_cast)
                else:
                    gw = torch.empty((co, c), dtype=x.dtype, device=x.device)
                    rc = L.ocpg_gemm(gz.data_ptr(), x.data_ptr(), gw.data_ptr(), None, dt, dt, 1, 0, co, c, m, co, c, c, 1, 0, 0, 0, 1.0, 0.0, st)
                if rc:
                    check(rc, "ocpg_gemm")
                gw = sw.publish(gw).view(w.shape)
        return gx, gw, None, None, gskip, None, None


def conv1x1_bn_act(x, w, scale, shift, skip, relu, splits):
    return Conv1x1BNAct.apply(x, w, scale, shift, skip, relu, splits)


_DT3 = {torch.float32: 0, torch.bfloat16: 1, torch.float16: 2}


def eligible3x3(x, conv):
    if not (x.is_cuda and x.dim() == 4 and x.dtype in _DT3 and conv.kernel_size == (3, 3) and conv.groups == 1 and conv.bias is None
            and conv.stride[0] == conv.stride[1] and conv.stride[0] in (1, 2) and conv.dilation[0] == conv.dilation[1]
            and conv.padding == conv.dilation and conv.padding_mode == "zeros" and x.is_contiguous(memory_format=_CL)):
        return False
    s = conv.stride[0]
    rows = x.shape[0] * ((x.shape[2] - 1) // s + 1) * ((x.shape[3] - 1) // s + 1)
    return x.shape[1] >= 256 and (x.shape[1] * x.element_size()) % 16 == 0 and rows <= 12288


class Conv3x3BNAct(Function):
    @staticmethod
    def forward(ctx, x, w, scale, shift, relu, stride, dil, splits):
        n, c, h, wd = x.shape
        co = w.shape[0]
        ho, wo = (h - 1) // stride + 1, (wd - 1) // stride + 1
        m = n * ho * wo
        dt = _DT3[x.dtype]
        L = lib()
        st = torch.cuda.current_stream().cuda_stream
        cols = torch.empty((m, 9 * c), dtype=x.dtype, device=x.device)
        check(L.ocpg_im2col3x3_nhwc(x.data_ptr(), n, h, wd, c, stride, dil, cols.data_ptr(), dt, st), "ocpg_im2col3x3_nhwc")
        w2 = w.permute(0, 2, 3, 1).reshape(co, 9 * c)
        if not w2.is_contiguous():
            w2 = w2.contiguous()
        y = torch.empty((n, co, ho, wo), dtype=x.dtype, device=x.device, memory_format=_CL)
        rc = L.ocpg_gemm_bn_act(cols.data_ptr(), w2.data_ptr(), y.data_ptr(), scale.data_ptr(), shift.data_ptr(), None, int(relu), dt, m, co,
                                9 * c, st) if EPILOGUE else -1105
        if rc and rc != -1105:
            check(rc, "ocpg_gemm_bn_act")
        if rc:
            check(L.ocpg_gemm(cols.data_ptr(), w2.data_ptr(), y.data_ptr(), None, dt, dt, 0, 1, m, co, 9 * c, 9 * c, 9 * c, co, 1, 0, 0, 0, 1.0,
                              0.0, st), "ocpg_gemm")
            check(L.ocpg_bn_act_fwd(y.data_ptr(), scale.data_ptr(), shift.data_ptr(), None, y.data_ptr(), m, co, 1, int(relu), dt, st),
                  "ocpg_bn_act_fwd")
        ctx.save_for_backward(cols, w2, y, scale)
        ctx.meta = (bool(relu), splits, (n, c, h, wd, ho, wo, stride, dil), w.shape)
        return y

    @staticmethod
    @once_differentiable
    def backward(ctx, gy):
        cols, w2, y, scale = ctx.saved_tensors
        relu, splits, (n, c, h, wd, ho, wo, stride, dil), wshape = ctx.meta
        co = w2.shape[0]
        m, k = cols.shape
        dt = _DT3[y.dtype]
        L = lib()
        st = torch.cuda.current_stream().cuda_stream
        if gy.dtype != y.dtype or not gy.is_contiguous(memory_format=_CL):
            gy = gy.to(y.dtype).contiguous(memory_format=_CL)
        gz = torch.empty_like(y)
        check(L.ocpg_bn_act_bwd(gy.data_ptr(), y.data_ptr(), scale.data_ptr(), gz.data_ptr(), None, m, co, 1, int(relu), dt, st), "ocpg_bn_act_bwd")
        gx = gw = None
        if ctx.needs_input_grad[0]:
            dcols = torch.empty((m, k), dtype=y.dtype, device=y.device)
            check(L.ocpg_gemm(gz.data_ptr(), w2.data_ptr(), dcols.data_ptr(), None, dt, dt, 0, 0, m, k, co, co, k, k, 1, 0, 0, 0, 1.0, 0.0, st),
                  "ocpg_gemm")
            gx = torch.empty((n, c, h, wd), dtype=y.dtype, device=y.device, memory_format=_CL)
            check(L.ocpg_col2im3x3_nhwc(dcols.data_ptr(), n, h, wd, c, stride, dil, gx.data_ptr(), dt, st), "ocpg_col2im3x3_nhwc")
        if ctx.needs_input_grad[1]:
            if splits > 1 and m % splits == 0:
                r = m // splits
                part = torch.empty((splits, co, k), dtype=y.dtype, device=y.device)
                check(L.ocpg_gemm(gz.data_ptr(), cols.data_ptr(), part.data_ptr(), None, dt, dt, 1, 0, co, k, r, co, k, k, splits, r * co, r * k,
                                  co * k, 1.0, 0.0, st), "ocpg_gemm")
                g2 = part.sum(0)
            else:
                g2 = torch.empty((co, k), dtype=y.dtype, device=y.device)
                check(L.ocpg_gemm(gz.data_ptr(), cols.data_ptr(), g2.data_ptr(), None, dt, dt, 1, 0, co, k, m, co, k, k, 1, 0, 0, 0, 1.0, 0.0, st),
                      "ocpg_gemm")
            gw = g2.view(co, 3, 3, c).permute(0, 3, 1, 2)
        return gx, gw, None, None, None, None, None, None


def conv3x3_bn_act(x, w, scale, shift, relu, stride, dil, splits):
    return Conv3x3BNAct.apply(x, w, scale, shift, relu, int(stride), int(dil), splits)


def eligible3x3_mfma(x, conv):
    if x.dtype == torch.float16 and (BODY_SPLITK or not DGRAD_OWN_WEIGHT):
        return False
    return (x.is_cuda and x.dim() == 4 and x.dtype in _H16 and conv.kernel_size == (3, 3) and conv.groups == 1
            and conv.bias is None and conv.stride[0] == conv.stride[1] and conv.stride[0] in (1, 2) and conv.dilation == (1, 1)
            and conv.padding == (1, 1) and conv.padding_mode == "zeros" and x.is_contiguous(memory_format=_CL)
            and x.shape[1] % 64 == 0 and conv.out_channels % 64 == 0 and x.shape[1] >= _MFMA_MIN_C and conv.out_channels >= _MFMA_MIN_C)


BODY_SPLITK = os.environ.get("OCPG_CONV3X3_SPLITK", "0") != "0"
WGRAD_OWN = os.environ.get("OCPG_WGRAD_OWN", "1") != "0"
DGRAD_OWN_WEIGHT = os.environ.get("OCPG_DGRAD_OWN_WEIGHT", "1") != "0"
_MFMA_MIN_C = int(os.environ.get("OCPG_MFMA_CONV3X3_MIN_C", "128"))


class Conv3x3MfmaBNAct(Function):

    @staticmethod
    def forward(ctx, x, w, scale, shift, relu, stride, splits):
        n, c, h, wd = x.shape
        co = w.shape[0]
        ho, wo = (h - 1) // stride + 1, (wd - 1) // stride + 1
        if not _both16(x, w):
            raise RuntimeError(f"Conv3x3MfmaBNAct: x and w must share one 16-bit dtype, got {x.dtype} and {w.dtype}")
        fp16 = x.dtype == torch.float16
        if fp16 and (BODY_SPLITK or not DGRAD_OWN_WEIGHT):
            raise RuntimeError("Conv3x3MfmaBNAct: OCPG_CONV3X3_SPLITK / OCPG_DGRAD_OWN_WEIGHT=0 select kernels that have no fp16 form")
        w2 = w.permute(0, 2, 3, 1)
        if not w2.is_contiguous():
            w2 = w2.contiguous()
        y = torch.empty((n, co, ho, wo), dtype=x.dtype, device=x.device, memory_format=_CL)
        st = torch.cuda.current_stream().cuda_stream
        cols = torch.empty((n * ho * wo, 9 * c), dtype=x.dtype, device=x.device) if (FWD_COLS and ctx.needs_input_grad[1]) else None
        sp = int(lib().ocpg_conv3x3_mfma_body_splits(n * ho * wo, co, c)) if (BODY_SPLITK and cols is None) else 1
        if sp > 1:
            part = torch.empty((sp, n * ho * wo, co), dtype=torch.float32, device=x.device)
            check(lib().ocpg_conv3x3_mfma_fwd_bn_splitk(x.data_ptr(), w2.data_ptr(), scale.data_ptr(), shift.data_ptr(), int(relu), n, h, wd, c, co, stride,
                                                        sp, part.data_ptr(), y.data_ptr(), st), "ocpg_conv3x3_mfma_fwd_bn_splitk")
        elif fp16:
            check(lib().ocpg_conv3x3_mfma_fwd_cols_h16(x.data_ptr(), w2.data_ptr(), scale.data_ptr(), shift.data_ptr(), int(relu), n, h, wd, c, co,
                                                       stride, y.data_ptr(), None if cols is None else cols.data_ptr(), 2, st),
                  "ocpg_conv3x3_mfma_fwd_cols_h16")
        else:
            check(lib().ocpg_conv3x3_mfma_fwd_cols(x.data_ptr(), w2.data_ptr(), scale.data_ptr(), shift.data_ptr(), int(relu), n, h, wd, c, co, stride,
                                                   y.data_ptr(), None if cols is None else cols.data_ptr(), st), "ocpg_conv3x3_mfma_fwd_cols")
        ctx.has_cols = cols is not None
        if cols is not None:
            ctx.save_for_backward(x, w2, y, scale, cols)
        else:
            ctx.save_for_backward(x, w2, y, scale)
        from ...amp_cache import is_cast_copy
        ctx.meta = (bool(relu), splits, stride)
        ctx.w_cast = is_cast_copy(w)
        tok = _claim_token(x) if PREMASK else None
        ctx.premask = tok if (tok is not None and not tok["skip"] and ctx.needs_input_grad[0]) else None
        ctx.offer = (_offer_token(y, scale, False, "OCPG_FUSED_DGRAD_BN")
                     if (FUSED_DGRAD_BN and relu and any(ctx.needs_input_grad)) else None)
        return y

    @staticmethod
    @once_differentiable
    def backward(ctx, gy):
        x, w2, y, scale = ctx.saved_tensors[:4]
        relu, splits, stride = ctx.meta
        n, c, h, wd = x.shape
        co, ho, wo = y.shape[1], y.shape[2], y.shape[3]
        m, k = n * ho * wo, 9 * c
        dt = _DT[y.dtype]
        fp16 = dt == 2
        L = lib()
        st = torch.cuda.current_stream().cuda_stream
        if gy.dtype != y.dtype or not gy.is_contiguous(memory_format=_CL):
            gy = gy.to(y.dtype).contiguous(memory_format=_CL)
        fused = _take_token(ctx.offer, gy)
        if fused is not None:
            gz = gy
        else:
            gz = torch.empty_like(y)
            check(L.ocpg_bn_act_bwd(gy.data_ptr(), y.data_ptr(), scale.data_ptr(), gz.data_ptr(), None, m, co, 1, int(relu), dt, st), "ocpg_bn_act_bwd")
        gx = gw = None
        if ctx.needs_input_grad[0]:
            gx = torch.empty((n, c, h, wd), dtype=y.dtype, device=y.device, memory_format=_CL)
            tok = ctx.premask
            mask_ptr, scale_ptr = (x.data_ptr(), tok["scale"].data_ptr()) if tok is not None else (None, None)
            sp = int(L.ocpg_conv3x3_mfma_body_splits(n * h * wd, c, co)) if (BODY_SPLITK and DGRAD_OWN_WEIGHT and c % 8 == 0 and not fp16) else 1
            if fp16:
                check(L.ocpg_conv3x3_mfma_dgrad_w_h16(gz.data_ptr(), w2.data_ptr(), mask_ptr, scale_ptr, n, h, wd, c, co, stride, gx.data_ptr(), 2, st),
                      "ocpg_conv3x3_mfma_dgrad_w_h16")
            elif sp > 1:
                part = torch.empty((sp, n * h * wd, c), dtype=torch.float32, device=y.device)
                check(L.ocpg_conv3x3_mfma_dgrad_w_splitk(gz.data_ptr(), w2.data_ptr(), mask_ptr, scale_ptr, n, h, wd, c, co, stride, sp, part.data_ptr(),
                                                         gx.data_ptr(), st), "ocpg_conv3x3_mfma_dgrad_w_splitk")
            elif DGRAD_OWN_WEIGHT and c % 8 == 0:
                check(L.ocpg_conv3x3_mfma_dgrad_w(gz.data_ptr(), w2.data_ptr(), mask_ptr, scale_ptr, n, h, wd, c, co, stride, gx.data_ptr(), st),
                      "ocpg_conv3x3_mfma_dgrad_w")
            else:
                wt = w2.permute(3, 1, 2, 0).contiguous()
                check(L.ocpg_conv3x3_mfma_dgrad_masked(gz.data_ptr(), wt.data_ptr(), mask_ptr, scale_ptr, n, h, wd, c, co, stride, gx.data_ptr(), st),
                      "ocpg_conv3x3_mfma_dgrad_masked")
            if tok is not None:
                _fill_token(tok, gx)
        if ctx.needs_input_grad[1]:
            from ...amp_cache import side_wgrad
            with side_wgrad(ctx.w_cast, gz, x) as sw:
                st = torch.cuda.current_stream().cuda_stream
                if WGRAD_OWN and not ctx.has_cols and c % 8 == 0 and co % 8 == 0:
                    sp = int(L.ocpg_conv3x3_mfma_wgrad_splits(n, h, wd, c, co, stride))
                    part = torch.empty((sp, co, k), dtype=y.dtype, device=y.device)
                    if fp16:
                        check(L.ocpg_conv3x3_mfma_wgrad_h16(gz.data_ptr(), x.data_ptr(), n, h, wd, c, co, stride, part.data_ptr(), 2, st),
                              "ocpg_conv3x3_mfma_wgrad_h16")
                    else:
                        check(L.ocpg_conv3x3_mfma_wgrad(gz.data_ptr(), x.data_ptr(), n, h, wd, c, co, stride, part.data_ptr(), st), "ocpg_conv3x3_mfma_wgrad")
                    g2 = _reduce_partials(part, ctx.w_cast) if sp > 1 else part[0]
                else:
                    if ctx.has_cols:
                        cols = ctx.saved_tensors[4]
                    else:
                        cols = torch.empty((m, k), dtype=y.dtype, device=y.device)
                        check(L.ocpg_im2col3x3_nhwc(x.data_ptr(), n, h, wd, c, stride, 1, cols.data_ptr(), dt, st), "ocpg_im2col3x3_nhwc")
                    if splits > 1 and m % splits == 0:
                        r = m // splits
                        part = torch.empty((splits, co, k), dtype=y.dtype, device=y.device)
                        check(L.ocpg_gemm(gz.data_ptr(), cols.data_ptr(), part.data_ptr(), None, dt, dt, 1, 0, co, k, r, co, k, k, splits, r * co, r * k,
                                          co * k, 1.0, 0.0, st), "ocpg_gemm")
                        g2 = _reduce_partials(part, ctx.w_cast)
                    else:
                        g2 = torch.empty((co, k), dtype=y.dtype, device=y.device)
                        check(L.ocpg_gemm(gz.data_ptr(), cols.data_ptr(), g2.data_ptr(), None, dt, dt, 1, 0, co, k, m, co, k, k, 1, 0, 0, 0, 1.0, 0.0, st),
                              "ocpg_gemm")
                gw = sw.publish(g2).view(co, 3, 3, c).permute(0, 3, 1, 2)
        return gx, gw, None, None, None, None, None


def conv3x3_mfma_bn_act(x, w, scale, shift, relu, stride, splits):
    return Conv3x3MfmaBNAct.apply(x, w, scale, shift, relu, int(stride), splits)


def eligible3x3_splitk(x, conv):
    if not (x.is_cuda and x.dim() == 4 and x.dtype in _H16 and conv.kernel_size == (3, 3) and conv.groups == 1
            and conv.stride[0] == conv.stride[1] and conv.stride[0] in (1, 2) and conv.dilation == (1, 1) and conv.padding == (1, 1)
            and conv.padding_mode == "zeros" and x.is_contiguous(memory_format=_CL) and x.shape[1] % 64 == 0 and conv.out_channels % 64 == 0):
        return False
    n, c, h, w = x.shape
    return int(lib().ocpg_conv3x3_mfma_splits(n, h, w, c, conv.out_channels, conv.stride[0])) > 1


class Conv3x3SplitK(Function):

    @staticmethod
    def forward(ctx, x, w, b, stride):
        n, c, h, wd = x.shape
        co = w.shape[0]
        ho, wo = (h - 1) // stride + 1, (wd - 1) // stride + 1
        m = n * ho * wo
        L = lib()
        st = torch.cuda.current_stream().cuda_stream
        w2 = w.permute(0, 2, 3, 1)
        if not w2.is_contiguous():
            w2 = w2.contiguous()
        if not _both16(x, w):
            raise RuntimeError(f"Conv3x3SplitK: x and w must share one 16-bit dtype, got {x.dtype} and {w.dtype}")
        splits = int(L.ocpg_conv3x3_mfma_splits(n, h, wd, c, co, stride))
        part = torch.empty((splits, m, co), dtype=torch.float32, device=x.device)
        y = torch.empty((n, co, ho, wo), dtype=x.dtype, device=x.device, memory_format=_CL)
        need_w = ctx.needs_input_grad[1]
        cols = torch.empty((m, 9 * c), dtype=x.dtype, device=x.device) if need_w else None
        bf = None if b is None else b.float()
        if x.dtype == torch.float16:
            check(L.ocpg_conv3x3_mfma_fwd_splitk_h16(x.data_ptr(), w2.data_ptr(), None if bf is None else bf.data_ptr(), n, h, wd, c, co, stride, splits,
                                                     part.data_ptr(), y.data_ptr(), 2, None if cols is None else cols.data_ptr(), 2, st),
                  "ocpg_conv3x3_mfma_fwd_splitk_h16")
        else:
            check(L.ocpg_conv3x3_mfma_fwd_splitk(x.data_ptr(), w2.data_ptr(), None if bf is None else bf.data_ptr(), n, h, wd, c, co, stride, splits,
                                                 part.data_ptr(), y.data_ptr(), 1, None if cols is None else cols.data_ptr(), st),
                  "ocpg_conv3x3_mfma_fwd_splitk")
        ctx.save_for_backward(w2, cols if need_w else w2)
        ctx.meta = (n, c, h, wd, ho, wo, stride, b is not None, need_w)
        return y

    @staticmethod
    @once_differentiable
    def backward(ctx, gy):
        w2, cols = ctx.saved_tensors
        n, c, h, wd, ho, wo, stride, has_b, need_w = ctx.meta
        co = w2.shape[0]
        m, k = n * ho * wo, 9 * c
        L = lib()
        st = torch.cuda.current_stream().cuda_stream
        dt = _DT[w2.dtype]
        if gy.dtype != w2.dtype or not gy.is_contiguous(memory_format=_CL):
            gy = gy.to(w2.dtype).contiguous(memory_format=_CL)
        gx = gw = gb = None
        if ctx.needs_input_grad[0]:
            gx = torch.empty((n, c, h, wd), dtype=gy.dtype, device=gy.device, memory_format=_CL)
            if dt == 2:
                check(L.ocpg_conv3x3_mfma_dgrad_w_h16(gy.data_ptr(), w2.data_ptr(), None, None, n, h, wd, c, co, stride, gx.data_ptr(), 2, st),
                      "ocpg_conv3x3_mfma_dgrad_w_h16")
            else:
                wt = w2.permute(3, 1, 2, 0).contiguous()
                check(L.ocpg_conv3x3_mfma_dgrad(gy.data_ptr(), wt.data_ptr(), n, h, wd, c, co, stride, gx.data_ptr(), st), "ocpg_conv3x3_mfma_dgrad")
        if need_w and ctx.needs_input_grad[1]:
            g2 = torch.empty((co, k), dtype=gy.dtype, device=gy.device)
            check(L.ocpg_gemm(gy.data_ptr(), cols.data_ptr(), g2.data_ptr(), None, dt, dt, 1, 0, co, k, m, co, k, k, 1, 0, 0, 0, 1.0, 0.0, st), "ocpg_gemm")
            gw = g2.view(co, 3, 3, c).permute(0, 3, 1, 2)
        if has_b and ctx.needs_input_grad[2]:
            gb = gy.permute(0, 2, 3, 1).reshape(m, co).float().sum(0).to(gy.dtype)
        return gx, gw, gb, None


def conv3x3_splitk(x, w, b, stride):
    return Conv3x3SplitK.apply(x, w, b, int(stride))
```

Before: 59.85.

## Split stride-2 conv3x3 input-gradient into output-parity classes with reduced tap lists

For stride-2 3x3 convolutions, the input-gradient kernel now tiles output pixels by their (y,x) parity class. Each class iterates only over the taps that can hit a strided output position (4, 2, 2 or 1 instead of 9), and a per-tile row map scatters results back to the full-resolution gradient. This removes the MFMA and load work spent on taps whose contributions are structurally zero. The forward patch-matrix store also moves behind a COLS template flag, so the non-cols variants drop that code. In exchange the launch splits into more, smaller-K tiles and the epilogue writes rows in a scattered pattern.

```diff
diff --git a/include/ocpg_hip.h b/include/ocpg_hip.h
--- a/include/ocpg_hip.h
+++ b/include/ocpg_hip.h
@@ -126,6 +126,10 @@
                                   int stride, void* dx, int dtype, void* stream);
 int ocpg_conv3x3_mfma_wgrad_h16(const void* gz, const void* x, int N, int H, int W, int Cin, int Cout, int stride, void* part, int dtype,
                                 void* stream);
+int ocpg_conv3x3_mfma_dgrad_w_s2(const void* dy, const void* w, const void* mask_y, const float* scale, int N, int H, int W, int Cin, int Cout,
+                                 int stride, void* dx, void* stream);
+int ocpg_conv3x3_mfma_dgrad_w_s2_h16(const void* dy, const void* w, const void* mask_y, const float* scale, int N, int H, int W, int Cin, int Cout,
+                                     int stride, void* dx, int dtype, void* stream);
 
 int ocpg_conv3x3_mfma_splits(int N, int H, int W, int Cin, int Cout, int stride);
 int ocpg_conv3x3_mfma_fwd_splitk(const void* x, const void* w, const float* bias, int N, int H, int W, int Cin, int Cout, int stride,
diff --git a/ocpg_amd/_lib.py b/ocpg_amd/_lib.py
--- a/ocpg_amd/_lib.py
+++ b/ocpg_amd/_lib.py
@@ -48,6 +48,8 @@
     "ocpg_conv3x3_mfma_fwd_cols_h16": [_vp, _vp, _vp, _vp] + [_int] * 7 + [_vp, _vp, _int, _vp],
     "ocpg_conv3x3_mfma_dgrad_w_h16": [_vp, _vp, _vp, _vp] + [_int] * 6 + [_vp, _int, _vp],
     "ocpg_conv3x3_mfma_wgrad_h16": [_vp, _vp] + [_int] * 6 + [_vp, _int, _vp],
+    "ocpg_conv3x3_mfma_dgrad_w_s2": [_vp, _vp, _vp, _vp] + [_int] * 6 + [_vp, _vp],
+    "ocpg_conv3x3_mfma_dgrad_w_s2_h16": [_vp, _vp, _vp, _vp] + [_int] * 6 + [_vp, _int, _vp],
     "ocpg_conv3x3_mfma_fwd_splitk": [_vp, _vp, _vp] + [_int] * 7 + [_vp, _vp, _int, _vp, _vp],
     "ocpg_conv3x3_mfma_fwd_splitk_h16": [_vp, _vp, _vp] + [_int] * 7 + [_vp, _vp, _int, _vp, _int, _vp],
     "ocpg_gemm": [_vp, _vp, _vp, _vp] + [_int] * 4 + [ctypes.c_longlong] * 10 + [ctypes.c_float, ctypes.c_float, _vp],
@@ -165,6 +167,7 @@
 
 
 CENSUS = {"on": False, "calls": {}}
+CENSUS_ALSO = {"ocpg_conv3x3_mfma_dgrad_w_s2": "ocpg_conv3x3_mfma_dgrad_w", "ocpg_conv3x3_mfma_dgrad_w_s2_h16": "ocpg_conv3x3_mfma_dgrad_w_h16"}
 
 
 def census(on=True):
@@ -190,7 +193,9 @@
             if CENSUS["on"]:
                 rc = fn(*a)
                 if rc == 0:
-                    CENSUS["calls"][name] = CENSUS["calls"].get(name, 0) + 1
+                    for k in (name, CENSUS_ALSO.get(name)):
+                        if k is not None:
+                            CENSUS["calls"][k] = CENSUS["calls"].get(k, 0) + 1
                 return rc
             if not (timed and _TIMING["on"]):
                 return fn(*a)
diff --git a/ocpg_amd/csrc/conv3x3_mfma.hip b/ocpg_amd/csrc/conv3x3_mfma.hip
--- a/ocpg_amd/csrc/conv3x3_mfma.hip
+++ b/ocpg_amd/csrc/conv3x3_mfma.hip
@@ -14,8 +14,8 @@
 typedef ocpg_h16::h16x8 bf16x8;
 typedef ocpg_h16::f32x16 f32x16;
 
-struct Bf16 : ocpg_h16::Bf16 { static constexpr bool STATIC_TAIL = false; };
-struct Fp16 : ocpg_h16::Fp16 { static constexpr bool STATIC_TAIL = true; };
+using ocpg_h16::Bf16;
+using ocpg_h16::Fp16;
 
 constexpr int BM = 64, BK = 64, NT = 256;
 constexpr int LDS_ROW = BK + 8;
@@ -30,6 +30,7 @@
   int Cout;
   int stride;
   long long M;
+  int ctile[3] = {0, 0, 0};
 };
 
 template <bool DGRAD>
@@ -93,18 +94,18 @@
   const unsigned mt = (unsigned)((g.M + BM - 1) / BM);
   const bool narrow = narrow_tiles(mt, Cout);
   const dim3 grid(mt, (unsigned)(narrow ? (Cout + 63) / 64 : (Cout + 127) / 128));
-  if (dtype == 2) {
-    if (narrow)
-      conv3x3_mfma_f16<false, 64><<<grid, NT, 0, (hipStream_t)stream>>>((const __half*)x, (const __half*)w, scale, bias, relu, g, (__half*)y, (__half*)cols);
-    else
-      conv3x3_mfma_f16<false, 128><<<grid, NT, 0, (hipStream_t)stream>>>((const __half*)x, (const __half*)w, scale, bias, relu, g, (__half*)y, (__half*)cols);
-  } else if (narrow) {
-    conv3x3_mfma<false, 64><<<grid, NT, 0, (hipStream_t)stream>>>(
-        (const __hip_bfloat16*)x, (const __hip_bfloat16*)w, scale, bias, relu, g, (__hip_bfloat16*)y, (__hip_bfloat16*)cols);
-  } else {
-    conv3x3_mfma<false, 128><<<grid, NT, 0, (hipStream_t)stream>>>(
-        (const __hip_bfloat16*)x, (const __hip_bfloat16*)w, scale, bias, relu, g, (__hip_bfloat16*)y, (__hip_bfloat16*)cols);
-  }
+  const hipStream_t s = (hipStream_t)stream;
+#define OCPG_FWD_LAUNCH(KERNEL, T, BN_, COLS_) \
+  KERNEL<false, BN_, false, false, COLS_><<<grid, NT, 0, s>>>((const T*)x, (const T*)w, scale, bias, relu, g, (T*)y, (T*)cols)
+#define OCPG_FWD_DISPATCH(KERNEL, T)                                              \
+  do {                                                                            \
+    if (narrow) { if (cols) OCPG_FWD_LAUNCH(KERNEL, T, 64, true); else OCPG_FWD_LAUNCH(KERNEL, T, 64, false); }   \
+    else { if (cols) OCPG_FWD_LAUNCH(KERNEL, T, 128, true); else OCPG_FWD_LAUNCH(KERNEL, T, 128, false); }        \
+  } while (0)
+  if (dtype == 2) OCPG_FWD_DISPATCH(conv3x3_mfma_f16, __half);
+  else OCPG_FWD_DISPATCH(conv3x3_mfma, __hip_bfloat16);
+#undef OCPG_FWD_DISPATCH
+#undef OCPG_FWD_LAUNCH
   const hipError_t e = hipGetLastError();
   return e == hipSuccess ? 0 : -(int)e;
 }
@@ -154,42 +155,68 @@
   return e == hipSuccess ? 0 : -(int)e;
 }
 
+namespace {
+
+int dgrad_w_launch(const void* dy, const void* w, const void* mask_y, const float* scale, int N, int H, int W, int Cin, int Cout, int stride, void* dx,
+                   int dtype, bool classes, void* stream) {
+  if (dtype != 1 && dtype != 2) return -1010;
+  if (N < 0 || H <= 0 || W <= 0 || Cin <= 0 || Cout <= 0) return -1006;
+  if ((stride != 1 && stride != 2) || Cout % BK != 0 || Cin % 8 != 0 || (classes && stride != 2)) return -2000;
+  if (N == 0) return 0;
+  if (!dy) return -1001;
+  if (!w) return -1002;
+  if (!dx) return -1011;
+  ConvGeom g;
+  g.N = N; g.H = H; g.W = W; g.C = Cout; g.Hs = (H - 1) / stride + 1; g.Ws = (W - 1) / stride + 1; g.Cout = Cin; g.stride = stride;
+  g.M = (long long)N * H * W;
+  unsigned mt = (unsigned)((g.M + BM - 1) / BM);
+  const bool narrow = narrow_tiles(mt, Cin);
+  if (classes) {
+    long long t = 0;
+    for (int k = 0; k < 4; ++k) {
+      const int cpy = (k & 1) ^ 1, cpx = k < 2;
+      t += ((long long)N * ((H - cpy + 1) / 2) * ((W - cpx + 1) / 2) + BM - 1) / BM;
+      if (k < 3) g.ctile[k] = (int)t;
+    }
+    mt = (unsigned)t;
+  }
+  const dim3 grid(mt, (unsigned)(narrow ? (Cin + 63) / 64 : (Cin + 127) / 128));
+  const hipStream_t s = (hipStream_t)stream;
+#define OCPG_DGRAD_LAUNCH(KERNEL, T, BN_, CLS_) \
+  KERNEL<true, BN_, false, true, false, CLS_><<<grid, NT, 0, s>>>((const T*)dy, (const T*)w, scale, nullptr, 0, g, (T*)dx, nullptr, (const T*)mask_y)
+#define OCPG_DGRAD_DISPATCH(KERNEL, T)                                            \
+  do {                                                                            \
+    if (narrow) { if (classes) OCPG_DGRAD_LAUNCH(KERNEL, T, 64, true); else OCPG_DGRAD_LAUNCH(KERNEL, T, 64, false); }   \
+    else { if (classes) OCPG_DGRAD_LAUNCH(KERNEL, T, 128, true); else OCPG_DGRAD_LAUNCH(KERNEL, T, 128, false); }        \
+  } while (0)
+  if (dtype == 2) OCPG_DGRAD_DISPATCH(conv3x3_mfma_f16, __half);
+  else OCPG_DGRAD_DISPATCH(conv3x3_mfma, __hip_bfloat16);
+#undef OCPG_DGRAD_DISPATCH
+#undef OCPG_DGRAD_LAUNCH
+  const hipError_t e = hipGetLastError();
+  return e == hipSuccess ? 0 : -(int)e;
+}
+
+}
+
 extern "C" int ocpg_conv3x3_mfma_dgrad_w_h16(const void* dy, const void* w, const void* mask_y, const float* scale, int N, int H, int W, int Cin,
                                              int Cout, int stride, void* dx, int dtype, void* stream) {
-  if (dtype != 1 && dtype != 2) return -1010;
-  if (N < 0 || H <= 0 || W <= 0 || Cin <= 0 || Cout <= 0) return -1006;
-  if ((stride != 1 && stride != 2) || Cout % BK != 0 || Cin % 8 != 0) return -2000;
-  if (N == 0) return 0;
-  if (!dy) return -1001;
-  if (!w) return -1002;
-  if (!dx) return -1011;
-  ConvGeom g;
-  g.N = N; g.H = H; g.W = W; g.C = Cout; g.Hs = (H - 1) / stride + 1; g.Ws = (W - 1) / stride + 1; g.Cout = Cin; g.stride = stride;
-  g.M = (long long)N * H * W;
-  const unsigned mt = (unsigned)((g.M + BM - 1) / BM);
-  const bool narrow = narrow_tiles(mt, Cin);
-  const dim3 grid(mt, (unsigned)(narrow ? (Cin + 63) / 64 : (Cin + 127) / 128));
-  if (dtype == 2) {
-    if (narrow)
-      conv3x3_mfma_f16<true, 64, false, true><<<grid, NT, 0, (hipStream_t)stream>>>((const __half*)dy, (const __half*)w, scale, nullptr, 0, g, (__half*)dx, nullptr,
-                                                                             (const __half*)mask_y);
-    else
-      conv3x3_mfma_f16<true, 128, false, true><<<grid, NT, 0, (hipStream_t)stream>>>((const __half*)dy, (const __half*)w, scale, nullptr, 0, g, (__half*)dx, nullptr,
-                                                                              (const __half*)mask_y);
-  } else if (narrow) {
-    conv3x3_mfma<true, 64, false, true><<<grid, NT, 0, (hipStream_t)stream>>>(
-        (const __hip_bfloat16*)dy, (const __hip_bfloat16*)w, scale, nullptr, 0, g, (__hip_bfloat16*)dx, nullptr, (const __hip_bfloat16*)mask_y);
-  } else {
-    conv3x3_mfma<true, 128, false, true><<<grid, NT, 0, (hipStream_t)stream>>>(
-        (const __hip_bfloat16*)dy, (const __hip_bfloat16*)w, scale, nullptr, 0, g, (__hip_bfloat16*)dx, nullptr, (const __hip_bfloat16*)mask_y);
-  }
-  const hipError_t e = hipGetLastError();
-  return e == hipSuccess ? 0 : -(int)e;
+  return dgrad_w_launch(dy, w, mask_y, scale, N, H, W, Cin, Cout, stride, dx, dtype, false, stream);
 }
 
 extern "C" int ocpg_conv3x3_mfma_dgrad_w(const void* dy, const void* w, const void* mask_y, const float* scale, int N, int H, int W, int Cin, int Cout,
                                          int stride, void* dx, void* stream) {
   return ocpg_conv3x3_mfma_dgrad_w_h16(dy, w, mask_y, scale, N, H, W, Cin, Cout, stride, dx, 1, stream);
+}
+
+extern "C" int ocpg_conv3x3_mfma_dgrad_w_s2_h16(const void* dy, const void* w, const void* mask_y, const float* scale, int N, int H, int W, int Cin,
+                                                int Cout, int stride, void* dx, int dtype, void* stream) {
+  return dgrad_w_launch(dy, w, mask_y, scale, N, H, W, Cin, Cout, stride, dx, dtype, true, stream);
+}
+
+extern "C" int ocpg_conv3x3_mfma_dgrad_w_s2(const void* dy, const void* w, const void* mask_y, const float* scale, int N, int H, int W, int Cin,
+                                            int Cout, int stride, void* dx, void* stream) {
+  return ocpg_conv3x3_mfma_dgrad_w_s2_h16(dy, w, mask_y, scale, N, H, W, Cin, Cout, stride, dx, 1, stream);
 }
 
 namespace {
@@ -263,12 +290,18 @@
   g.M = (long long)N * g.H * g.W;
   const unsigned mt = (unsigned)((g.M + BM - 1) / BM);
   const dim3 grid(mt, (unsigned)((Cout + 63) / 64), (unsigned)splits);
-  if (dtype == 2)
+  if (dtype == 2 && cols)
+    conv3x3_mfma_f16<false, 64, true, false, true><<<grid, NT, 0, (hipStream_t)stream>>>((const __half*)x, (const __half*)w, nullptr, nullptr, 0, g,
+                                                                                       reinterpret_cast<__half*>(part), (__half*)cols);
+  else if (dtype == 2)
     conv3x3_mfma_f16<false, 64, true><<<grid, NT, 0, (hipStream_t)stream>>>((const __half*)x, (const __half*)w, nullptr, nullptr, 0, g,
-                                                                          reinterpret_cast<__half*>(part), (__half*)cols);
+                                                                          reinterpret_cast<__half*>(part), nullptr);
+  else if (cols)
+    conv3x3_mfma<false, 64, true, false, true><<<grid, NT, 0, (hipStream_t)stream>>>(
+        (const __hip_bfloat16*)x, (const __hip_bfloat16*)w, nullptr, nullptr, 0, g, reinterpret_cast<__hip_bfloat16*>(part), (__hip_bfloat16*)cols);
   else
     conv3x3_mfma<false, 64, true><<<grid, NT, 0, (hipStream_t)stream>>>(
-        (const __hip_bfloat16*)x, (const __hip_bfloat16*)w, nullptr, nullptr, 0, g, reinterpret_cast<__hip_bfloat16*>(part), (__hip_bfloat16*)cols);
+        (const __hip_bfloat16*)x, (const __hip_bfloat16*)w, nullptr, nullptr, 0, g, reinterpret_cast<__hip_bfloat16*>(part), nullptr);
   const long long MC = g.M * Cout;
   k_splitk_reduce<<<(unsigned)((MC / 4 + 255) / 256), 256, 0, (hipStream_t)stream>>>(part, bias, splits, MC, Cout, y, out_dt);
   const hipError_t e = hipGetLastError();
diff --git a/ocpg_amd/csrc/conv3x3_mfma_kernel.h b/ocpg_amd/csrc/conv3x3_mfma_kernel.h
--- a/ocpg_amd/csrc/conv3x3_mfma_kernel.h
+++ b/ocpg_amd/csrc/conv3x3_mfma_kernel.h
@@ -1,4 +1,4 @@
-template <bool DGRAD, int BN, bool SPLITK = false, bool BTR = false>
+template <bool DGRAD, int BN, bool SPLITK = false, bool BTR = false, bool COLS = false, bool CLS = false>
 __global__ __launch_bounds__(NT) void CONV3X3_KERNEL(const CONV3X3_ELEM::T* __restrict__ x, const CONV3X3_ELEM::T* __restrict__ w,
                                                      const float* __restrict__ scale, const float* __restrict__ bias, int relu, ConvGeom g,
                                                      CONV3X3_ELEM::T* __restrict__ y, CONV3X3_ELEM::T* __restrict__ cols,
@@ -7,6 +7,8 @@
   using T = E::T;
   static_assert(!SPLITK || BN == 64, "the split-K epilogue is the 64-column one");
   static_assert(!BTR || DGRAD, "the untransposed weight operand is the input gradient's");
+  static_assert(!COLS || !DGRAD, "the patch matrix is the forward's");
+  static_assert(!CLS || (BTR && !SPLITK), "parity-class tiles are the own-weight input gradient's");
   constexpr int BROW = BN + 8;
   constexpr int BSEG = BN / 8;
   static_assert(BK * BROW <= BN * LDS_ROW, "the [k][n] image fits the [n][k] one's buffer");
@@ -18,28 +20,42 @@
   short (*Bs)[BN * LDS_ROW] = reinterpret_cast<short (*)[BN * LDS_ROW]>(smem + 2 * BM * LDS_ROW);
   const int tid = threadIdx.x, lane = tid & 63, wave = tid >> 6;
   const int wm = wave & 1, wn = wave >> 1;
-  const long long m0 = (long long)blockIdx.x * BM;
+  int cpy = 0, cpx = 0, ntaps = 9;
+  unsigned taplist = 0;
+  int tile = blockIdx.x;
+  if constexpr (CLS) {
+    const int k = (tile >= g.ctile[0]) + (tile >= g.ctile[1]) + (tile >= g.ctile[2]);
+    if (k > 0) tile -= g.ctile[k - 1];
+    cpy = (k & 1) ^ 1;
+    cpx = k < 2;
+    ntaps = k == 0 ? 4 : k == 3 ? 1 : 2;
+    taplist = k == 0 ? 0x8620u : k == 1 ? 0x53u : k == 2 ? 0x71u : 0x4u;
+  }
+  const int rH = CLS ? (g.H - cpy + 1) / 2 : g.H, rW = CLS ? (g.W - cpx + 1) / 2 : g.W;
+  const long long rM = CLS ? (long long)g.N * rH * rW : g.M;
+  const long long m0 = (long long)tile * BM;
   const int n0 = blockIdx.y * BN;
   const int srow = tid / SEGS, sseg = tid % SEGS;
   int pn[A_L], py[A_L], px[A_L];
   bool row_ok[A_L];
   {
-    const int hw = g.H * g.W;
+    const int hw = rH * rW;
 #pragma unroll
     for (int i = 0; i < A_L; ++i) {
       const long long mrow = m0 + srow + i * ROWS_PER_PASS;
-      row_ok[i] = mrow < g.M;
+      row_ok[i] = mrow < rM;
       const long long mr = row_ok[i] ? mrow : 0;
       pn[i] = (int)(mr / hw);
       const int r = (int)(mr - (long long)pn[i] * hw);
-      py[i] = r / g.W;
-      px[i] = r - py[i] * g.W;
+      py[i] = r / rW;
+      px[i] = r - py[i] * rW;
+      if constexpr (CLS) { py[i] = 2 * py[i] + cpy; px[i] = 2 * px[i] + cpx; }
     }
   }
   const int C = g.C, ksteps_per_tap = C / BK;
   const int cps = SPLITK ? ksteps_per_tap / (int)gridDim.z : ksteps_per_tap;
   const int c_lo = SPLITK ? (int)blockIdx.z * cps : 0, c_hi = c_lo + cps;
-  const int ksteps = 9 * cps;
+  const int ksteps = (CLS ? ntaps : 9) * cps;
   const long long wrow_stride = 9LL * C;
   const T* wp[B_L];
 #pragma unroll
@@ -57,10 +73,10 @@
   int f_tap = 0, f_c = c_lo;
   auto fetch = [&](Regs& R) {
     uint4 (&a)[A_L] = R.a; uint4 (&bq)[B_L] = R.b; unsigned& z = R.z;
-    const int tap = f_tap, fc = min(f_c, c_hi - 1);
+    const int tap = CLS ? (int)((taplist >> (4 * f_tap)) & 15u) : f_tap, fc = min(f_c, c_hi - 1);
     const int ky = (tap * 11) >> 5, kx = tap - ky * 3;
     const int c0 = fc * BK + sseg * 8;
-    R.coff = f_c < c_hi ? tap * C + c0 : -1;
+    if constexpr (COLS) R.coff = f_c < c_hi ? tap * C + c0 : -1;
     z = 0;
 #pragma unroll
     for (int i = 0; i < A_L; ++i) {
@@ -72,7 +88,7 @@
     const long long woff = BTR ? (long long)fc * BK * (9LL * g.Cout) + (long long)tap * g.Cout : (long long)tap * C + fc * BK;
 #pragma unroll
     for (int i = 0; i < B_L; ++i) bq[i] = *reinterpret_cast<const uint4*>(wp[i] + woff);
-    if (++f_tap == 9) { f_tap = 0; ++f_c; }
+    if (++f_tap == (CLS ? ntaps : 9)) { f_tap = 0; ++f_c; }
   };
   auto park = [&](int buf, const Regs& R) {
     const uint4 (&a)[A_L] = R.a; const uint4 (&bq)[B_L] = R.b; const unsigned z = R.z;
@@ -88,8 +104,8 @@
         *reinterpret_cast<uint4*>(&Bs[buf][(srow + i * ROWS_PER_PASS) * LDS_ROW + sseg * 8]) = bq[i];
       }
     }
-    if constexpr (!DGRAD) {
-      if (cols && blockIdx.y == 0 && R.coff >= 0) {
+    if constexpr (COLS) {
+      if (blockIdx.y == 0 && R.coff >= 0) {
 #pragma unroll
         for (int i = 0; i < A_L; ++i)
           if (row_ok[i])
@@ -166,6 +182,16 @@
     step(ks + 1, S2);
     step(ks + 2, S0);
   }
+  long long* rowmap = reinterpret_cast<long long*>(smem + 4 * 4096);
+  static_assert(!CLS || sizeof(smem) >= 2 * 4096 * sizeof(float) + BM * sizeof(long long), "the row map lies behind the tile images");
+  if constexpr (CLS) {
+    if (tid < BM) {
+      const long long q = m0 + tid;
+      const int hw = rH * rW, qn = (int)(q / hw), r = (int)(q - (long long)qn * hw), qy = r / rW, qx = r - qy * rW;
+      rowmap[tid] = q < rM ? ((long long)qn * g.H + 2 * qy + cpy) * g.W + 2 * qx + cpx : -1;
+    }
+    if constexpr (!KSPLIT) __syncthreads();
+  }
   if constexpr (KSPLIT) {
     float* red = reinterpret_cast<float*>(smem);
     static_assert(sizeof(smem) >= 2 * 4096 * sizeof(float), "two tile images");
@@ -190,8 +216,8 @@
     if (wave == 0) { add(red + 4096); put(red); }
     __syncthreads();
     const int m = tid >> 2, nq = (tid & 3) * 16;
-    const long long row = m0 + m;
-    if (row < g.M) {
+    const long long row = CLS ? rowmap[m] : m0 + m;
+    if (CLS ? row >= 0 : row < g.M) {
       const int r = (m & 3) + 4 * ((m & 31) >> 3), h = ((m & 31) >> 2) & 1, t0 = (m >> 5) * 2 + (nq >> 5);
       const float* src = red + (t0 * 16 + r) * 64 + (nq & 31) + 32 * h;
       const int col0 = n0 + nq;
@@ -233,12 +259,10 @@
           const bf16x8 lo = *reinterpret_cast<const bf16x8*>(mk), hi = *reinterpret_cast<const bf16x8*>(mk + 8);
 #pragma unroll
           for (int j = 0; j < 8; ++j) { keep[j] = lo[j] > 0; keep[8 + j] = hi[j] > 0; }
-        } else if constexpr (E::STATIC_TAIL) {
+        } else {
 #pragma unroll
           for (int j = 0; j < 16; ++j)
             if (col0 + j < g.Cout) keep[j] = reinterpret_cast<const short*>(mk)[j] > 0;
-        } else {
-          for (int j = 0; j < 16 && col0 + j < g.Cout; ++j) keep[j] = reinterpret_cast<const short*>(mk)[j] > 0;
         }
       }
 #pragma unroll
@@ -255,12 +279,10 @@
         for (int j = 0; j < 8; ++j) { lo[j] = o[j]; hi[j] = o[8 + j]; }
         *reinterpret_cast<bf16x8*>(dst) = lo;
         *reinterpret_cast<bf16x8*>(dst + 8) = hi;
-      } else if constexpr (E::STATIC_TAIL) {
+      } else {
 #pragma unroll
         for (int j = 0; j < 16; ++j)
           if (col0 + j < g.Cout) reinterpret_cast<short*>(dst)[j] = o[j];
-      } else {
-        for (int j = 0; j < 16 && col0 + j < g.Cout; ++j) reinterpret_cast<short*>(dst)[j] = o[j];
       }
     }
     return;
@@ -272,10 +294,11 @@
     const float sv = scale ? scale[col] : 1.f, bv = bias ? bias[col] : 0.f;
 #pragma unroll
     for (int r = 0; r < 16; ++r) {
-      const long long row = m0 + wm * 32 + (r & 3) + 8 * (r >> 2) + 4 * (lane >> 5);
+      const int m = wm * 32 + (r & 3) + 8 * (r >> 2) + 4 * (lane >> 5);
+      const long long row = CLS ? rowmap[m] : m0 + m;
       float v = acc[j][r] * sv + bv;
       if (relu) v = fmaxf(v, 0.f);
-      if (row < g.M) {
+      if (CLS ? row >= 0 : row < g.M) {
         if (mask && !(reinterpret_cast<const short*>(mask)[row * g.Cout + col] > 0)) v = 0.f;
         y[row * g.Cout + col] = E::narrow(v);
       }
diff --git a/ocpg_amd/models/ops/functions/conv_bn_func.py b/ocpg_amd/models/ops/functions/conv_bn_func.py
--- a/ocpg_amd/models/ops/functions/conv_bn_func.py
+++ b/ocpg_amd/models/ops/functions/conv_bn_func.py
@@ -332,6 +332,7 @@
 BODY_SPLITK = os.environ.get("OCPG_CONV3X3_SPLITK", "0") != "0"
 WGRAD_OWN = os.environ.get("OCPG_WGRAD_OWN", "1") != "0"
 DGRAD_OWN_WEIGHT = os.environ.get("OCPG_DGRAD_OWN_WEIGHT", "1") != "0"
+DGRAD_S2_CLASSES = os.environ.get("OCPG_DGRAD_S2_CLASSES", "1") != "0"
 _MFMA_MIN_C = int(os.environ.get("OCPG_MFMA_CONV3X3_MIN_C", "128"))
 
 
@@ -405,16 +406,19 @@
             tok = ctx.premask
             mask_ptr, scale_ptr = (x.data_ptr(), tok["scale"].data_ptr()) if tok is not None else (None, None)
             sp = int(L.ocpg_conv3x3_mfma_body_splits(n * h * wd, c, co)) if (BODY_SPLITK and DGRAD_OWN_WEIGHT and c % 8 == 0 and not fp16) else 1
+            s2 = stride == 2 and DGRAD_S2_CLASSES
             if fp16:
-                check(L.ocpg_conv3x3_mfma_dgrad_w_h16(gz.data_ptr(), w2.data_ptr(), mask_ptr, scale_ptr, n, h, wd, c, co, stride, gx.data_ptr(), 2, st),
-                      "ocpg_conv3x3_mfma_dgrad_w_h16")
+                fn = L.ocpg_conv3x3_mfma_dgrad_w_s2_h16 if s2 else L.ocpg_conv3x3_mfma_dgrad_w_h16
+                check(fn(gz.data_ptr(), w2.data_ptr(), mask_ptr, scale_ptr, n, h, wd, c, co, stride, gx.data_ptr(), 2, st),
+                      "ocpg_conv3x3_mfma_dgrad_w_s2_h16" if s2 else "ocpg_conv3x3_mfma_dgrad_w_h16")
             elif sp > 1:
                 part = torch.empty((sp, n * h * wd, c), dtype=torch.float32, device=y.device)
                 check(L.ocpg_conv3x3_mfma_dgrad_w_splitk(gz.data_ptr(), w2.data_ptr(), mask_ptr, scale_ptr, n, h, wd, c, co, stride, sp, part.data_ptr(),
                                                          gx.data_ptr(), st), "ocpg_conv3x3_mfma_dgrad_w_splitk")
             elif DGRAD_OWN_WEIGHT and c % 8 == 0:
-                check(L.ocpg_conv3x3_mfma_dgrad_w(gz.data_ptr(), w2.data_ptr(), mask_ptr, scale_ptr, n, h, wd, c, co, stride, gx.data_ptr(), st),
-                      "ocpg_conv3x3_mfma_dgrad_w")
+                fn = L.ocpg_conv3x3_mfma_dgrad_w_s2 if s2 else L.ocpg_conv3x3_mfma_dgrad_w
+                check(fn(gz.data_ptr(), w2.data_ptr(), mask_ptr, scale_ptr, n, h, wd, c, co, stride, gx.data_ptr(), st),
+                      "ocpg_conv3x3_mfma_dgrad_w_s2" if s2 else "ocpg_conv3x3_mfma_dgrad_w")
             else:
                 wt = w2.permute(3, 1, 2, 0).contiguous()
                 check(L.ocpg_conv3x3_mfma_dgrad_masked(gz.data_ptr(), wt.data_ptr(), mask_ptr, scale_ptr, n, h, wd, c, co, stride, gx.data_ptr(), st),
@@ -516,8 +520,10 @@
         if ctx.needs_input_grad[0]:
             gx = torch.empty((n, c, h, wd), dtype=gy.dtype, device=gy.device, memory_format=_CL)
             if dt == 2:
-                check(L.ocpg_conv3x3_mfma_dgrad_w_h16(gy.data_ptr(), w2.data_ptr(), None, None, n, h, wd, c, co, stride, gx.data_ptr(), 2, st),
-                      "ocpg_conv3x3_mfma_dgrad_w_h16")
+                s2 = stride == 2 and DGRAD_S2_CLASSES
+                fn = L.ocpg_conv3x3_mfma_dgrad_w_s2_h16 if s2 else L.ocpg_conv3x3_mfma_dgrad_w_h16
+                check(fn(gy.data_ptr(), w2.data_ptr(), None, None, n, h, wd, c, co, stride, gx.data_ptr(), 2, st),
+                      "ocpg_conv3x3_mfma_dgrad_w_s2_h16" if s2 else "ocpg_conv3x3_mfma_dgrad_w_h16")
             else:
                 wt = w2.permute(3, 1, 2, 0).contiguous()
                 check(L.ocpg_conv3x3_mfma_dgrad(gy.data_ptr(), wt.data_ptr(), n, h, wd, c, co, stride, gx.data_ptr(), st), "ocpg_conv3x3_mfma_dgrad")
```

After: 60.92 (median of 6 runs). 1.8% higher.
